# Dyfine/SimCLR_pytorch_distributed

Hardware: AMD Instinct MI355X
Metric: images/sec (whole node) SimCLR ResNet-50 BS=256; CIFAR-10 linear-probe top-1 (higher is better)
Workload: dtype bf16; 1 GPU; model=resnet50 (CIFAR stem) + MLP head 2048-2048-128, SimCLR tau=0.5, global_batch=256, per_gpu_batch=256, views=2, image_size=32, parallelism=dp1, backend=native, syncbn_transport=none, hip_graph=False, loss_steps=254

## Files before the change

csrc/bindings/block_ops.cpp:

```cpp
#include "ops_decl.h"
#include "conv_internal.h"
#include "launchers.h"

namespace sdx_bind {
namespace {

using sdx_plan::knobs;

enum BlockSlot { kOut = 0, kX = 0, kY1, kA1, kY2, kA2, kY3, kYs, kMask, kSlots };
enum BnSlot { kSc = 0, kSh, kMu, kIv, kBnStride };

double rows_of(const torch::Tensor& y) { return (double)(y.numel() / y.size(3)); }

bool sub_addend_enabled() {
  static const bool on = sdx_plan::env_flag("SDX_SUB_ADDEND", true);
  return on;
}

bool dgrad_bnstat_enabled() {
  static const bool on = sdx_plan::env_flag("SDX_DGRAD_BNSTAT", true);
  return on;
}

DgradOpts into(OptT out, OptT addend, OptT addend_mask = {}, int64_t addend_sub = 0) {
  DgradOpts o;
  o.out = out; o.addend = addend; o.addend_mask = addend_mask; o.addend_sub = addend_sub;
  return o;
}

void side_wgrad(const torch::Tensor& dy, const torch::Tensor& x, int64_t R, int64_t S, int64_t stride, int64_t pad,
                const torch::Tensor& sink, int64_t side) {
  if (side == 0) {
    conv_wgrad(dy, x, R, S, stride, pad, 0, -1, sink, true, c10::nullopt, c10::nullopt);
    return;
  }
  auto guard = side_fork(side, dy.device(), {dy, x});
  if (splitk_merge_enabled() && !splitk_deferring(cur_stream())) splitk_defer_begin(cur_stream());
  conv_wgrad(dy, x, R, S, stride, pad, 0, -1, sink, true, c10::nullopt, c10::nullopt);
}

std::vector<torch::Tensor> fold_gram_now(const torch::Tensor& a2) {
  const int64_t K3 = a2.size(3);
  auto opt = a2.options().dtype(at::kFloat);
  auto Sm = torch::empty({K3, 1, 1, K3}, opt);
  conv_wgrad(a2, a2, 1, 1, 1, 0, 0, -1, Sm, false, c10::nullopt, c10::nullopt);
  auto part = torch::empty({bnfold_colsum_blocks(), K3}, opt);
  auto cs = torch::empty({K3}, opt);
  check_hip(launch_bnfold_colsum(a2.data_ptr(), a2.numel() / K3, (int)K3, part.data_ptr<float>(), cs.data_ptr<float>(),
                                 cur_stream()),
            "bnfold_colsum");
  return {Sm, cs, part};
}

std::vector<torch::Tensor> fold_gram(torch::Tensor a2, int64_t side) {
  check_bf16_nhwc(a2, "a2");
  if (side == 0) return fold_gram_now(a2);
  auto guard = side_fork(side, a2.device(), {a2});
  return fold_gram_now(a2);
}

void side_fold_wgrad(const torch::Tensor& dz, const torch::Tensor& a2, const torch::Tensor& w3,
                     const torch::Tensor& coef, const torch::Tensor& sink, int64_t side,
                     const torch::Tensor* gram = nullptr, const torch::Tensor* Gpre = nullptr) {
  if (side != 0 && splitk_deferring(reinterpret_cast<hipStream_t>(side))) check_hip(splitk_flush(), "splitk_flush");
  const int64_t C3 = dz.size(3), K3 = a2.size(3);
  auto body = [&]() {
    auto opt = coef.options();
    torch::Tensor G;
    if (Gpre != nullptr) {
      G = *Gpre;
    } else {
      G = torch::empty({C3, 1, 1, K3}, opt);
      conv_wgrad(dz, a2, 1, 1, 1, 0, 0, -1, G, false, c10::nullopt, c10::nullopt);
    }
    torch::Tensor Sm, cs, part;
    if (gram != nullptr) {
      Sm = gram[0];
      cs = gram[1];
    } else {
      auto g3 = fold_gram_now(a2);
      Sm = g3[0];
      cs = g3[1];
      part = g3[2];
    }
    check_hip(launch_bnfold_wgrad(coef.data_ptr<float>(), G.data_ptr<float>(), Sm.data_ptr<float>(),
                                  cs.data_ptr<float>(), 1, w3.data_ptr(), (int)C3, (int)K3, sink.data_ptr<float>(),
                                  1, cur_stream()),
              "bnfold_wgrad");
    if (side != 0) {
      side_stash().push_back(G);
      side_stash().push_back(Sm);
      side_stash().push_back(cs);
      if (part.defined()) side_stash().push_back(part);
    }
  };
  if (side == 0) {
    body();
    return;
  }
  auto guard = side_fork(side, dz.device(), {dz, a2, w3, coef});
  body();
}

struct FoldOps {
  torch::Tensor w;
  torch::Tensor t;
  torch::Tensor bias;
  bool cat = false;
  DgradOpts dgrad_opts(const torch::Tensor& a2) const {
    DgradOpts o;
    if (cat) {
      o.cat = &a2;
      o.cat_bias = &bias;
    } else {
      o.addend = t;
      o.add_pre = true;
    }
    return o;
  }
};
bool fold_cat_enabled() {
  static const bool on = sdx_plan::env_flag("SDX_FOLD_CAT", true);
  return on;
}
FoldOps fold_dgrad_operands(const torch::Tensor& coef, const torch::Tensor& w3, const torch::Tensor& wt3,
                            const torch::Tensor& a2, const torch::Tensor& mu, const torch::Tensor* gram) {
  const int64_t C3 = w3.size(0), K3 = w3.size(3);
  TORCH_CHECK(w3.size(1) == 1 && w3.size(2) == 1 && wt3.size(0) == K3 && wt3.size(3) == C3 && a2.size(3) == K3 &&
                  coef.numel() == 3 * C3,
              "bn3 fold: conv3 must be 1x1 [C][1][1][K] with a2 of K channels");
  const int64_t rows = a2.numel() / K3;
  TORCH_CHECK(rows < (1LL << 31), "bn3 fold: too many rows");
  check_vec(mu, C3, "fold mu");
  const ConvGeom gd = conv_geom(a2.size(0), a2.size(1), a2.size(2), K3, C3, 1, 1, 1, 0);
  FoldOps r;
  r.bias = torch::empty({K3}, coef.options());
  const float* cs = gram != nullptr ? gram[1].data_ptr<float>() : nullptr;
  if (fold_cat_enabled() && sdx_plan::dgrad_cat_supported(gd, (int)K3, knobs())) {
    r.cat = true;
    r.w = torch::empty({K3, 1, 1, C3 + K3}, w3.options());
    uint16_t* wc = reinterpret_cast<uint16_t*>(r.w.data_ptr());
    check_hip(launch_bnfold_prep(coef.data_ptr<float>(), w3.data_ptr(), wt3.data_ptr(), (int)C3, (int)K3, wc, wc + C3,
                                 r.bias.data_ptr<float>(), mu.data_ptr<float>(), cs, (long)rows, cur_stream(),
                                 (int)(C3 + K3), (int)(C3 + K3)),
              "bnfold_prep");
    return r;
  }
  r.w = torch::empty_like(wt3);
  auto mx = torch::empty({K3, 1, 1, K3}, w3.options());
  check_hip(launch_bnfold_prep(coef.data_ptr<float>(), w3.data_ptr(), wt3.data_ptr(), (int)C3, (int)K3, r.w.data_ptr(),
                               mx.data_ptr(), r.bias.data_ptr<float>(), mu.data_ptr<float>(), cs, (long)rows,
                               cur_stream()),
            "bnfold_prep");
  const ConvGeom g = conv_geom(rows, 1, 1, K3, K3, 1, 1, 1, 0);
  r.t = torch::empty_like(a2);
  const GemmEpi epi{r.bias.data_ptr<float>(), 0, 0};
  check_hip(launch_conv_fwd(g, a2.data_ptr(), mx.data_ptr(), r.t.data_ptr(), nullptr, auto_cfg(rows, K3, K3, true),
                            cur_stream(), nullptr, nullptr, &epi),
            "bnfold T gemm");
  return r;
}

std::vector<torch::Tensor> block_fwd(torch::Tensor x, std::vector<torch::Tensor> w, std::vector<torch::Tensor> bn,
                                     int64_t stride, bool bottleneck, bool proj, bool training, double eps,
                                     double momentum, int64_t comm, bool fold_fwd = false, int64_t side = 0) {
  const int nconv = bottleneck ? 3 : 2;
  TORCH_CHECK((int)w.size() == nconv + (proj ? 1 : 0), "block_fwd: weight count");
  TORCH_CHECK(bn.size() == w.size() * 4, "block_fwd: 4 BN tensors per conv");
  auto bn_fwd = [&](int i, const torch::Tensor& slab, double count) {
    return bn_forward(slab, count, bn[i * 4], bn[i * 4 + 1], bn[i * 4 + 2], bn[i * 4 + 3], eps, momentum, training,
                      comm);
  };
  auto conv_bn = [&](const torch::Tensor& in, int i, int64_t s, int64_t p) -> std::pair<torch::Tensor, BnState> {
    auto c = conv_fwd(in, w[i], s, p, training, -1, c10::nullopt, c10::nullopt);
    return {c[0], bn_fwd(i, c[1], rows_of(c[0]))};
  };
  auto relu_bn = [](const torch::Tensor& y, const BnState& s) {
    return bn_apply(y, s.sc, s.sh, {}, true, c10::nullopt);
  };
  std::vector<BnState> st;
  std::vector<torch::Tensor> out(kMask);
  torch::Tensor ys_side, slab_side;
  hipEvent_t sc_done = nullptr;
  if (proj && training && side != 0) {
    const torch::Tensor& ws = w[nconv];
    check_bf16_nhwc(x, "x");
    check_bf16_nhwc(ws, "w_shortcut");
    TORCH_CHECK(ws.size(3) == x.size(3) && ws.size(1) == 1 && ws.size(2) == 1, "block_fwd: 1x1 shortcut");
    const ConvGeom gs = fwd_geom(x, ws, stride, 0);
    const int64_t M = (int64_t)gs.N * gs.P * gs.Q;
    const int cfg = auto_cfg(M, gs.K, gs.C, true);
    ys_side = torch::empty({gs.N, gs.P, gs.Q, gs.K}, x.options());
    slab_side = torch::empty({sdx_plan::cdiv(M, sdx_plan::tile_m(cfg)), 2, gs.K}, x.options().dtype(at::kFloat));
    auto guard = side_fork(side, x.device(), {});
    check_hip(launch_conv_fwd(gs, x.data_ptr(), ws.data_ptr(), ys_side.data_ptr(), slab_side.data_ptr<float>(), cfg,
                              cur_stream()),
              "block_fwd shortcut conv (side stream)");
    sc_done = stream_mark();
  }
  const int64_t s1 = bottleneck ? 1 : stride, p1 = bottleneck ? 0 : 1;
  auto c1 = conv_bn(x, 0, s1, p1);
  st.push_back(c1.second);
  auto a1 = relu_bn(c1.first, st[0]);
  const int64_t s2 = bottleneck ? stride : 1;
  auto c2 = conv_bn(a1, 1, s2, 1);
  st.push_back(c2.second);
  torch::Tensor last = c2.first, a2;
  int lastbn = 1;
  fold_fwd = fold_fwd && bottleneck && training && w[2].size(1) == 1 && w[2].size(2) == 1 &&
             (proj || (stride == 1 && w[2].size(0) == x.size(3))) && sdx_plan::fwd_bnapply_supported(knobs());
  torch::Tensor o, ys;
  auto shortcut = [&] {
    if (sc_done != nullptr) {
      stream_wait(sc_done);
      st.push_back(bn_fwd(nconv, slab_side, rows_of(ys_side)));
      ys = ys_side;
    } else {
      auto cs = conv_bn(x, nconv, stride, 0);
      st.push_back(cs.second);
      ys = cs.first;
    }
  };
  torch::Tensor omask;
  if (bottleneck) {
    a2 = relu_bn(c2.first, st[1]);
    if (fold_fwd) {
      auto c3s = conv_fwd(a2, w[2], 1, 0, true, -1, c10::nullopt, c10::nullopt, nullptr, true);
      st.push_back(bn_fwd(2, c3s[1], rows_of(a2)));
      GemmEpi epi{};
      epi.bn_scale = st[2].sc.data_ptr<float>();
      epi.bn_shift = st[2].sh.data_ptr<float>();
      if (proj) {
        shortcut();
        TORCH_CHECK(ys.size(0) == a2.size(0) && ys.size(1) == a2.size(1) && ys.size(2) == a2.size(2) &&
                        ys.size(3) == w[2].size(0),
                    "block_fwd: shortcut output shape");
        epi.resid = ys.data_ptr();
        epi.resid_scale = st[3].sc.data_ptr<float>();
        epi.resid_shift = st[3].sh.data_ptr<float>();
      } else {
        epi.resid = x.data_ptr();
      }
      omask = torch::empty({rows_of(a2) * w[2].size(0) / 8}, x.options().dtype(at::kByte));
      epi.mask_out = omask.data_ptr<uint8_t>();
      o = conv_fwd(a2, w[2], 1, 0, false, -1, c10::nullopt, c10::nullopt, &epi)[0];
      last = torch::Tensor();
    } else {
      auto c3 = conv_bn(a2, 2, 1, 0);
      st.push_back(c3.second);
      last = c3.first;
    }
    lastbn = 2;
  }
  if (training && !omask.defined())
    omask = torch::empty({last.numel() / 8}, last.options().dtype(at::kByte));
  const OptT om = training ? OptT(omask) : OptT();
  if (fold_fwd) {
  } else if (proj) {
    shortcut();
    o = bn_apply(last, st[lastbn].sc, st[lastbn].sh, {ys, st[nconv].sc, st[nconv].sh, 1}, true, om);
  } else {
    o = bn_apply(last, st[lastbn].sc, st[lastbn].sh, {x, {}, {}, 2}, true, om);
  }
  out.push_back(omask);
  out[kOut] = o;
  out[kY1] = c1.first;
  out[kA1] = a1;
  out[kY2] = c2.first;
  out[kA2] = bottleneck ? a2 : torch::Tensor();
  out[kY3] = bottleneck ? last : torch::Tensor();
  out[kYs] = ys;
  for (auto& b : st) {
    out.push_back(b.sc);
    out.push_back(b.sh);
    out.push_back(b.mu);
    out.push_back(b.iv);
  }
  return out;
}

std::vector<torch::Tensor> block_bwd(torch::Tensor dout, std::vector<torch::Tensor> saved,
                                     std::vector<torch::Tensor> bnst, std::vector<torch::Tensor> wt,
                                     std::vector<torch::Tensor> dw, std::vector<torch::Tensor> bng, int64_t stride,
                                     bool bottleneck, bool proj, int64_t side, int64_t comm, OptT in_slab,
                                     std::vector<torch::Tensor> prev, std::vector<torch::Tensor> fold_w) {
  const int nconv = bottleneck ? 3 : 2;
  const int nbn = nconv + (proj ? 1 : 0);
  struct DeferGuard {
    bool ok = false;
    ~DeferGuard() {
      if (!ok) splitk_defer_cancel();
    }
  } defer_guard;
  TORCH_CHECK((int)wt.size() == nbn && (int)dw.size() == nbn && (int)bng.size() == 3 * nbn &&
                  (int)bnst.size() == kBnStride * nbn && saved.size() == kSlots,
              "block_bwd: argument counts");
  const torch::Tensor &x = saved[kX], &y1 = saved[kY1], &a1 = saved[kA1], &y2 = saved[kY2], &a2 = saved[kA2],
                      &y3 = saved[kY3], &ys = saved[kYs], &out = saved[kMask];
  auto S = [&](int i, int k) { return bnst[i * kBnStride + k]; };
  auto bset = [&](int i) { return BnBwdSet{bng[i * 3], S(i, kMu), S(i, kIv), bng[i * 3 + 1], bng[i * 3 + 2]}; };
  const int64_t H = x.size(1), W = x.size(2);
  const int lastbn = nconv - 1;
  const torch::Tensor& ylast = bottleneck ? y3 : y2;
  const bool no_y3 = bottleneck && (!y3.defined() || y3.numel() == 0);
  const double cnt_last = rows_of(y2), cnt1 = rows_of(y1);
  torch::Tensor dylast, dys, dz;
  const bool have_slab = in_slab.has_value() && in_slab->defined() && in_slab->numel() > 0;
  if (have_slab) TORCH_CHECK(in_slab->size(1) == (proj ? 3 : 2), "block_bwd: in_slab set count");
  const size_t nfw = fold_w.size() == 3 || fold_w.size() == 6 ? fold_w.size() / 3 : fold_w.size();
  const bool grams = nfw != fold_w.size();
  const bool fold = bottleneck && have_slab && nfw >= 1 && nfw <= (proj ? 2u : 1u) && fold_w[0].defined() &&
                    (nfw == 1 || (stride == 1 && fold_w[1].defined()));
  const bool fold_sc = fold && proj && nfw == 2;
  TORCH_CHECK(!no_y3 || fold, "block_bwd: a forward-folded block needs its BN3 fold (next block's slab)");
  const torch::Tensor* gram3 = grams ? &fold_w[nfw] : nullptr;
  const torch::Tensor* grams_sc = grams && nfw == 2 ? &fold_w[nfw + 2] : nullptr;
  torch::Tensor coef3, coefs, Gfold;
  if (no_y3) {
    const int64_t C3 = dout.size(3), K3 = a2.size(3), ns = in_slab->size(1);
    TORCH_CHECK(in_slab->size(0) > 2 && in_slab->size(2) == C3 && fold_w[0].size(0) == C3 &&
                    fold_w[0].size(3) == K3,
                "block_bwd: forward-folded BN3 slab / weights");
    Gfold = torch::empty({C3, 1, 1, K3}, dout.options().dtype(at::kFloat));
    conv_wgrad(dout, a2, 1, 1, 1, 0, 0, -1, Gfold, false, c10::nullopt, c10::nullopt);
    float* rows = in_slab->data_ptr<float>() + (in_slab->size(0) - 2) * ns * C3;
    check_hip(launch_bnfold_rowdot(Gfold.data_ptr<float>(), fold_w[0].data_ptr(), (int)C3, (int)K3, (int)ns, rows,
                                   cur_stream()),
              "bnfold_rowdot");
  }
  {
    const BnBwdSrc src{dout, out, ylast, proj ? OptT(ys) : OptT()};
    auto c = bn_bwd_coefs(comm, have_slab ? nullptr : &src, have_slab ? &*in_slab : nullptr, cnt_last, bset(lastbn),
                          proj ? bset(nconv) : BnBwdSet{});
    if (fold) {
      coef3 = c[0];
      dz = dout;
      if (fold_sc)
        coefs = c[1];
      else if (proj)
        dys = bn_bwd_apply({dz, {}, ys}, c[1], c10::nullopt, false)[0];
    } else if (proj) {
      auto r = bn_bwd_apply(src, c[0], c[1], false);
      dylast = r[0];
      dys = r[1];
    } else {
      const bool bitmask = out.scalar_type() == at::kByte;
      auto r = bn_bwd_apply(src, c[0], c10::nullopt, !bitmask);
      dylast = r[0];
      dz = bitmask ? torch::Tensor() : r[2];
    }
  }
  auto dgrad_bn = [&](const torch::Tensor& dyo, const torch::Tensor& w, const torch::Tensor& y, int64_t st,
                      int64_t pad, int i, double cnt, const DgradOpts& o = {}) -> std::pair<torch::Tensor, torch::Tensor> {
    if (dgrad_bnstat_enabled()) {
      DgradStat ds;
      ds.ya = y; ds.ma = S(i, kMu); ds.msc = S(i, kSc); ds.msh = S(i, kSh);
      auto r = conv_dgrad_bnstat(dyo, w, y.size(1), y.size(2), st, pad, -1, o, ds);
      return {r[0], bn_bwd_coefs(comm, nullptr, &r[1], cnt, bset(i))[0]};
    }
    auto da = conv_dgrad(dyo, w, y.size(1), y.size(2), st, pad, -1, o);
    const BnBwdSrc src{da, {}, y, {}, S(i, kSc), S(i, kSh)};
    return {da, bn_bwd_coefs(comm, &src, nullptr, cnt, bset(i))[0]};
  };
  auto bn_relu_bwd = [&](const torch::Tensor& da, const torch::Tensor& y, const torch::Tensor& coef, int i) {
    return bn_bwd_apply({da, {}, y, {}, S(i, kSc), S(i, kSh)}, coef, c10::nullopt, false)[0];
  };
  torch::Tensor dy1;
  if (bottleneck) {
    std::pair<torch::Tensor, torch::Tensor> r2;
    if (fold) {
      auto op = fold_dgrad_operands(coef3, fold_w[0], wt[2], a2, S(lastbn, kMu), gram3);
      side_fold_wgrad(dz, a2, fold_w[0], coef3, dw[2], side, gram3, Gfold.defined() ? &Gfold : nullptr);
      r2 = dgrad_bn(dz, op.w, y2, 1, 0, 1, cnt_last, op.dgrad_opts(a2));
    } else {
      side_wgrad(dylast, a2, 1, 1, 1, 0, dw[2], side);
      r2 = dgrad_bn(dylast, wt[2], y2, 1, 0, 1, cnt_last);
    }
    auto dy2 = bn_relu_bwd(r2.first, y2, r2.second, 1);
    side_wgrad(dy2, a1, 3, 3, stride, 1, dw[1], side);
    auto r1 = dgrad_bn(dy2, wt[1], y1, stride, 1, 0, cnt1);
    dy1 = bn_relu_bwd(r1.first, y1, r1.second, 0);
    side_wgrad(dy1, x, 1, 1, 1, 0, dw[0], side);
  } else {
    side_wgrad(dylast, a1, 3, 3, 1, 1, dw[1], side);
    auto r1 = dgrad_bn(dylast, wt[1], y1, 1, 1, 0, cnt1);
    dy1 = bn_relu_bwd(r1.first, y1, r1.second, 0);
    side_wgrad(dy1, x, 3, 3, stride, 1, dw[0], side);
  }
  const int64_t s1 = bottleneck ? 1 : stride, p1 = bottleneck ? 0 : 1;
  const bool want_prev = dgrad_bnstat_enabled() && prev.size() >= 5 && prev[4].defined() && prev[4].numel() > 0;
  const bool prev_fold = want_prev && prev.size() >= 6 && prev[5].defined() && prev[5].numel() > 0;
  torch::Tensor prev_slab;
  auto last_dgrad = [&](const DgradOpts& o) -> torch::Tensor {
    if (!want_prev) return conv_dgrad(dy1, wt[0], H, W, s1, p1, -1, o);
    const bool two = prev[2].defined() && prev[2].numel() > 0;
    const bool prev_noy = !prev[0].defined() || prev[0].numel() == 0;
    TORCH_CHECK(!prev_noy || prev_fold, "block_bwd: previous block without y3 must fold");
    DgradStat ds;
    ds.ya = prev[0]; ds.ma = prev[1]; ds.mask_bits = prev[4];
    if (two) {
      ds.yb = prev[2];
      ds.mb = prev[3];
    }
    ds.store_masked = prev_fold ? 1 : 0;
    ds.extra_rows = prev_noy ? 2 : 0;
    auto r = conv_dgrad_bnstat(dy1, wt[0], H, W, s1, p1, -1, o, ds);
    prev_slab = r[1];
    return r[0];
  };
  torch::Tensor dx;
  if (fold_sc) {
    auto op = fold_dgrad_operands(coefs, fold_w[1], wt[nconv], x, S(nconv, kMu), grams_sc);
    side_fold_wgrad(dz, x, fold_w[1], coefs, dw[nconv], side, grams_sc);
    dx = conv_dgrad(dz, op.w, H, W, 1, 0, -1, op.dgrad_opts(x));
    dx = last_dgrad(into(dx, dx));
  } else if (proj) {
    side_wgrad(dys, x, 1, 1, stride, 0, dw[nconv], side);
    if (stride > 1 && sub_addend_enabled()) {
      auto dxs = conv_dgrad(dys, wt[nconv], dys.size(1), dys.size(2), 1, 0, -1);
      dx = last_dgrad(into({}, dxs, {}, stride));
    } else {
      dx = conv_dgrad(dys, wt[nconv], H, W, stride, 0, -1);
      dx = last_dgrad(into(dx, dx));
    }
  } else if (dz.defined()) {
    dx = last_dgrad(into({}, dz));
  } else {
    dx = last_dgrad(into({}, dout, out));
  }
  check_hip(splitk_flush(), "splitk_flush");
  defer_guard.ok = true;
  return {dx, prev_slab};
}


void check_f32(const torch::Tensor& t, int64_t numel, const char* name) {
  TORCH_CHECK(t.is_cuda() && t.scalar_type() == at::kFloat && t.is_contiguous() && t.numel() == numel, name,
              " must be a contiguous float32 GPU tensor of ", numel, " elements");
}

void check_bf16_flat(const torch::Tensor& t, const char* name) {
  TORCH_CHECK(t.is_cuda() && t.scalar_type() == at::kBFloat16 && t.is_contiguous(), name,
              " must be a contiguous bf16 GPU tensor");
}

std::pair<int64_t, int64_t> fold_weight_dims(const torch::Tensor& w) {
  check_bf16_flat(w, "w");
  TORCH_CHECK(w.dim() == 4 && w.size(1) == 1 && w.size(2) == 1 && w.size(0) > 0 && w.size(3) > 0 &&
                  w.size(0) < (1 << 20) && w.size(3) < (1 << 20),
              "w must be [C][1][1][K]");
  return {w.size(0), w.size(3)};
}

void bnfold_prep_test(torch::Tensor coef, torch::Tensor w, torch::Tensor wt, OptT mu, OptT cs, int64_t rows,
                      int64_t ldw, int64_t ldm, torch::Tensor wd_out, torch::Tensor mx_out, torch::Tensor bias_out) {
  const auto [C, K] = fold_weight_dims(w);
  check_bf16_flat(wt, "wt");
  TORCH_CHECK(wt.dim() == 4 && wt.size(0) == K && wt.size(1) == 1 && wt.size(2) == 1 && wt.size(3) == C,
              "wt must be [K][1][1][C]");
  check_f32(coef, 3 * C, "coef");
  check_f32(bias_out, K, "bias_out");
  check_bf16_flat(wd_out, "wd_out");
  check_bf16_flat(mx_out, "mx_out");
  TORCH_CHECK(rows >= 0 && rows < (1LL << 31) && ldw >= 0 && ldm >= 0 && ldw < (1 << 24) && ldm < (1 << 24),
              "bnfold_prep: rows, ldw or ldm out of range");
  const int64_t lw = ldw == 0 ? C : ldw, lm = ldm == 0 ? K : ldm;
  TORCH_CHECK(wd_out.numel() >= (K - 1) * lw + C, "wd_out too small for K rows of ldw");
  TORCH_CHECK(mx_out.numel() >= (K - 1) * lm + K, "mx_out too small for K rows of ldm");
  const float* pmu = opt_ptr(mu, C, "mu");
  const float* pcs = opt_ptr(cs, K, "cs");
  c10::DeviceGuard dg(w.device());
  check_hip(launch_bnfold_prep(coef.data_ptr<float>(), w.data_ptr(), wt.data_ptr(), (int)C, (int)K, wd_out.data_ptr(),
                               mx_out.data_ptr(), bias_out.data_ptr<float>(), pmu, pcs, (long)rows, cur_stream(),
                               (int)ldw, (int)ldm),
            "bnfold_prep");
}

std::vector<torch::Tensor> bnfold_colsum_test(torch::Tensor x, OptT partial) {
  check_bf16_flat(x, "x");
  TORCH_CHECK(x.dim() == 2 && x.size(1) > 0 && x.numel() < (1LL << 31), "x must be [rows][K] bf16");
  TORCH_CHECK(reinterpret_cast<uintptr_t>(x.data_ptr()) % 16 == 0, "x must be 16-byte aligned");
  const int64_t rows = x.size(0), K = x.size(1);
  c10::DeviceGuard dg(x.device());
  auto opt = x.options().dtype(at::kFloat);
  const int64_t nb = bnfold_colsum_blocks();
  torch::Tensor part = partial.has_value() && partial->defined() ? *partial : torch::empty({nb, K}, opt);
  check_f32(part, nb * K, "partial");
  auto cs = torch::empty({K}, opt);
  check_hip(launch_bnfold_colsum(x.data_ptr(), (long)rows, (int)K, part.data_ptr<float>(), cs.data_ptr<float>(),
                                 cur_stream()),
            "bnfold_colsum");
  return {cs, part};
}

torch::Tensor bnfold_wgrad_test(torch::Tensor coef, torch::Tensor G, torch::Tensor S, torch::Tensor cs,
                                torch::Tensor w, torch::Tensor sink, bool accumulate) {
  const auto [C, K] = fold_weight_dims(w);
  check_f32(coef, 3 * C, "coef");
  check_f32(G, C * K, "G");
  check_f32(S, K * K, "S");
  check_f32(sink, C * K, "sink");
  TORCH_CHECK(cs.dim() == 2 && cs.size(1) == K, "cs must be [ncs][K]");
  check_f32(cs, cs.size(0) * K, "cs");
  c10::DeviceGuard dg(w.device());
  check_hip(launch_bnfold_wgrad(coef.data_ptr<float>(), G.data_ptr<float>(), S.data_ptr<float>(), cs.data_ptr<float>(),
                                (int)cs.size(0), w.data_ptr(), (int)C, (int)K, sink.data_ptr<float>(),
                                accumulate ? 1 : 0, cur_stream()),
            "bnfold_wgrad");
  return sink;
}

torch::Tensor bnfold_rowdot_test(torch::Tensor G, torch::Tensor w, int64_t ns, torch::Tensor out) {
  const auto [C, K] = fold_weight_dims(w);
  check_f32(G, C * K, "G");
  TORCH_CHECK(ns >= 0 && ns <= 16 && out.dim() == 3 && out.size(0) == 2 && out.size(1) == ns && out.size(2) == C,
              "out must be [2][ns][C]");
  check_f32(out, 2 * ns * C, "out");
  c10::DeviceGuard dg(w.device());
  check_hip(launch_bnfold_rowdot(G.data_ptr<float>(), w.data_ptr(), (int)C, (int)K, (int)ns, out.data_ptr<float>(),
                                 cur_stream()),
            "bnfold_rowdot");
  return out;
}

}

void register_block(pybind11::module& m) {
  m.def("bnfold_prep", &bnfold_prep_test, "BN3 fold (test only): Wd, Mx and b into caller-supplied outputs",
        pybind11::arg("coef"), pybind11::arg("w"), pybind11::arg("wt"), pybind11::arg("mu") = pybind11::none(),
        pybind11::arg("cs") = pybind11::none(), pybind11::arg("rows") = 0, pybind11::arg("ldw") = 0,
        pybind11::arg("ldm") = 0, pybind11::arg("wd_out"), pybind11::arg("mx_out"), pybind11::arg("bias_out"));
  m.def("bnfold_colsum", &bnfold_colsum_test, "BN3 fold (test only): column sums of x [rows][K] -> (cs, partial)",
        pybind11::arg("x"), pybind11::arg("partial") = pybind11::none());
  m.def("bnfold_wgrad", &bnfold_wgrad_test, "BN3 fold (test only): the folded weight gradient into sink",
        pybind11::arg("coef"), pybind11::arg("G"), pybind11::arg("S"), pybind11::arg("cs"), pybind11::arg("w"),
        pybind11::arg("sink"), pybind11::arg("accumulate"));
  m.def("bnfold_rowdot", &bnfold_rowdot_test, "BN3 fold (test only): Σ_k W·G as fp32 hi / lo slab rows",
        pybind11::arg("G"), pybind11::arg("w"), pybind11::arg("ns"), pybind11::arg("out"));
  m.def("side_stash_release", [] { side_stash().clear(); },
        "drop the tensors kept alive for side-stream wgrads (after join)");
  m.def("block_fwd", &block_fwd, "native residual-block forward (whole kernel sequence; comm: SyncBN handle or 0)",
        pybind11::arg("x"), pybind11::arg("w"), pybind11::arg("bn"), pybind11::arg("stride"),
        pybind11::arg("bottleneck"), pybind11::arg("proj"), pybind11::arg("training"), pybind11::arg("eps"),
        pybind11::arg("momentum"), pybind11::arg("comm") = 0, pybind11::arg("fold_fwd") = false,
        pybind11::arg("side") = 0);
  m.def("fold_gram", &fold_gram,
        "BN3 fold: [a2ᵀ·a2, Σ_rows a2, scratch] of a folded conv's input, issued on the side stream",
        pybind11::arg("a2"), pybind11::arg("side"));
  m.def("block_bwd", &block_bwd, "native residual-block backward (dgrad chain + side-stream wgrads)",
        pybind11::arg("dout"), pybind11::arg("saved"), pybind11::arg("bnst"), pybind11::arg("wt"),
        pybind11::arg("dw"), pybind11::arg("bng"), pybind11::arg("stride"), pybind11::arg("bottleneck"),
        pybind11::arg("proj"), pybind11::arg("side"), pybind11::arg("comm") = 0,
        pybind11::arg("in_slab") = pybind11::none(), pybind11::arg("prev") = std::vector<torch::Tensor>(),
        pybind11::arg("fold_w") = std::vector<torch::Tensor>());
}

}
```

csrc/bindings/bn_ops.cpp:

```cpp
#include "ops_decl.h"
#include "conv_internal.h"
#include "launchers.h"

#include <map>
#include <mutex>
#include <utility>

namespace sdx_bind {

unsigned* reduce_counters(const torch::Device& dev, int nslots) {
  constexpr int kSlots = 256, kPerSlot = 64;
  TORCH_CHECK(nslots >= 1 && nslots <= kXgmiMaxPeers, "counter slots");
  static std::mutex mu;
  static std::map<int, std::pair<torch::Tensor, int>> pool;
  std::lock_guard<std::mutex> lk(mu);
  auto& e = pool[dev.index()];
  if (!e.first.defined())
    e.first = torch::zeros({kSlots * kPerSlot}, torch::TensorOptions().dtype(at::kInt).device(dev));
  int slot = e.second;
  if (slot + nslots > kSlots) slot = 0;
  e.second = (slot + nslots) % kSlots;
  return reinterpret_cast<unsigned*>(e.first.data_ptr<int>()) + slot * kPerSlot;
}

torch::Tensor reduce_scratch(const torch::Tensor& like, int64_t rows, int64_t nsets, int64_t C, int z) {
  return torch::empty({z * col_reduce_gy((int)rows) * nsets * C}, like.options().dtype(at::kDouble));
}

FusedX fused_exchange(int64_t comm) {
  FusedX f;
  if (comm != 0) f.on = small_comm_fused(comm, &f.x);
  return f;
}

namespace {

struct SyncPlan {
  int world = 1;
  FusedX fx;
  bool rccl() const { return world > 1 && !fx.on; }
  const FusedX* fused() const { return fx.on ? &fx : nullptr; }
};
SyncPlan sync_plan(int64_t comm) {
  SyncPlan p;
  p.world = small_comm_world(comm);
  if (p.world > 1) p.fx = fused_exchange(comm);
  return p;
}

void check_slab(const torch::Tensor& slab, int64_t nsets) {
  TORCH_CHECK(slab.is_cuda() && slab.scalar_type() == at::kFloat && slab.dim() == 3 && slab.size(1) == nsets &&
                  slab.is_contiguous(),
              "slab must be [rows, ", nsets, ", C] float32");
  TORCH_CHECK(slab.size(2) <= 4096, "C <= 4096");
}

torch::Tensor bn_stats_reduce(torch::Tensor slab) {
  check_slab(slab, 2);
  c10::DeviceGuard dg(slab.device());
  const int64_t rows = slab.size(0), C = slab.size(2);
  auto out = torch::empty({2, C}, slab.options().dtype(at::kDouble));
  auto scratch = reduce_scratch(slab, rows, 2, C);
  check_hip(launch_col_reduce(slab.data_ptr<float>(), rows, 2, C, scratch.data_ptr<double>(),
                              reduce_counters(slab.device()), out.data_ptr<double>(), 0, nullptr, nullptr,
                              cur_stream()),
            "bn_stats_reduce");
  return out;
}

struct FinalizeOut {
  torch::Tensor scale, shift, mean, invstd;
};

BnFinalizeArgs finalize_args(const torch::Tensor& like, int64_t C, double count, const OptT& gamma, const OptT& beta,
                             double eps, double momentum, bool update, const OptT& running_mean,
                             const OptT& running_var, FinalizeOut& o) {
  BnFinalizeArgs a{};
  a.count = count;
  a.gamma = opt_ptr(gamma, C, "gamma");
  a.beta = opt_ptr(beta, C, "beta");
  a.eps = (float)eps;
  a.momentum = (float)momentum;
  a.update_running = update ? 1 : 0;
  if (update) {
    TORCH_CHECK(running_mean.has_value() && running_var.has_value(), "running stats required for update");
    check_vec(*running_mean, C, "running_mean");
    check_vec(*running_var, C, "running_var");
    a.running_mean = running_mean->data_ptr<float>();
    a.running_var = running_var->data_ptr<float>();
  }
  auto fo = like.options().dtype(at::kFloat);
  o.scale = torch::empty({C}, fo);
  o.shift = torch::empty({C}, fo);
  o.mean = torch::empty({C}, fo);
  o.invstd = torch::empty({C}, fo);
  a.scale = o.scale.data_ptr<float>();
  a.shift = o.shift.data_ptr<float>();
  a.mean = o.mean.data_ptr<float>();
  a.invstd = o.invstd.data_ptr<float>();
  return a;
}

std::vector<torch::Tensor> bn_finalize(torch::Tensor sums, double count, OptT gamma, OptT beta, double eps,
                                       double momentum, bool update, OptT running_mean, OptT running_var) {
  TORCH_CHECK(sums.is_cuda() && sums.scalar_type() == at::kDouble && sums.dim() == 2 && sums.size(0) == 2 &&
                  sums.is_contiguous(),
              "sums must be [2, C] float64");
  const int64_t C = sums.size(1);
  c10::DeviceGuard dg(sums.device());
  FinalizeOut o;
  const BnFinalizeArgs a =
      finalize_args(sums, C, count, gamma, beta, eps, momentum, update, running_mean, running_var, o);
  check_hip(launch_bn_finalize(sums.data_ptr<double>(), C, a, cur_stream()), "bn_finalize");
  return {o.scale, o.shift, o.mean, o.invstd};
}

std::vector<torch::Tensor> bn_stats_finalize(torch::Tensor slab, double count, OptT gamma, OptT beta, double eps,
                                             double momentum, bool update, OptT running_mean, OptT running_var,
                                             const FusedX* fx = nullptr) {
  check_slab(slab, 2);
  c10::DeviceGuard dg(slab.device());
  const int64_t rows = slab.size(0), C = slab.size(2);
  FinalizeOut o;
  const BnFinalizeArgs a =
      finalize_args(slab, C, count, gamma, beta, eps, momentum, update, running_mean, running_var, o);
  auto sums = torch::empty({2, C}, slab.options().dtype(at::kDouble));
  const int z = fx ? fx->z() : 1;
  auto scratch = reduce_scratch(slab, rows, 2, C, z);
  check_hip(launch_col_reduce(slab.data_ptr<float>(), rows, 2, C, scratch.data_ptr<double>(),
                              reduce_counters(slab.device(), z), sums.data_ptr<double>(), 1, &a, nullptr, cur_stream(),
                              fx ? fx->p() : nullptr),
            "bn_stats_finalize");
  return {o.scale, o.shift, o.mean, o.invstd};
}

std::vector<torch::Tensor> bn_eval_affine(OptT gamma, OptT beta, torch::Tensor rm, torch::Tensor rv, double eps) {
  const int64_t C = rm.numel();
  check_vec(rm, C, "running_mean");
  check_vec(rv, C, "running_var");
  c10::DeviceGuard dg(rm.device());
  auto scale = torch::empty({C}, rm.options()), shift = torch::empty({C}, rm.options());
  check_hip(launch_bn_eval_affine(C, opt_ptr(gamma, C, "gamma"), opt_ptr(beta, C, "beta"), rm.data_ptr<float>(),
                                  rv.data_ptr<float>(), (float)eps, scale.data_ptr<float>(), shift.data_ptr<float>(),
                                  cur_stream()),
            "bn_eval_affine");
  return {scale, shift};
}

}

BnState bn_forward(const torch::Tensor& slab, double count, const torch::Tensor& g, const torch::Tensor& b,
                   const torch::Tensor& rm, const torch::Tensor& rv, double eps, double mom, bool training,
                   int64_t comm) {
  if (!training) {
    auto r = bn_eval_affine(g, b, rm, rv, eps);
    return {r[0], r[1], torch::Tensor(), torch::Tensor()};
  }
  const SyncPlan sp = sync_plan(comm);
  std::vector<torch::Tensor> r;
  if (sp.rccl()) {
    auto sums = bn_stats_reduce(slab);
    small_all_reduce_(comm, sums);
    r = bn_finalize(sums, count * sp.world, g, b, eps, mom, true, rm, rv);
  } else {
    r = bn_stats_finalize(slab, count * sp.world, g, b, eps, mom, true, rm, rv, sp.fused());
    if (sp.fx.on) small_comm_fused_issued(comm);
  }
  return {r[0], r[1], r[2], r[3]};
}

torch::Tensor bn_apply(torch::Tensor y, torch::Tensor scale, torch::Tensor shift, const BnResidual& res, bool relu,
                       OptT mask_out) {
  check_bf16_nhwc(y, "y");
  const int64_t C = y.size(3);
  check_vec(scale, C, "scale");
  check_vec(shift, C, "shift");
  const void* rp = nullptr;
  const float *s2 = nullptr, *t2 = nullptr;
  TORCH_CHECK(res.mode >= 0 && res.mode <= 2, "res_mode");
  if (res.mode != 0) {
    TORCH_CHECK(res.r.has_value(), "residual tensor required");
    check_bf16_nhwc(*res.r, "residual");
    TORCH_CHECK(res.r->sizes() == y.sizes(), "residual shape mismatch");
    rp = res.r->data_ptr();
    if (res.mode == 1) {
      s2 = opt_ptr(res.scale2, C, "scale2");
      t2 = opt_ptr(res.shift2, C, "shift2");
      TORCH_CHECK(s2 && t2, "scale2/shift2 required for res_mode 1");
    }
  }
  c10::DeviceGuard dg(y.device());
  auto out = torch::empty_like(y);
  void* mp = nullptr;
  if (mask_out.has_value()) {
    check_mask(*mask_out, y.numel(), "mask_out");
    mp = mask_out->data_ptr();
  }
  check_hip(launch_bn_apply(y.data_ptr(), scale.data_ptr<float>(), shift.data_ptr<float>(), rp, s2, t2, (int)res.mode,
                            relu ? 1 : 0, out.data_ptr(), y.numel(), C, cur_stream(), mp),
            "bn_apply");
  return out;
}

namespace {

void check_bwd_C(int64_t C) {
  TORCH_CHECK(C <= 2048 && (C & (C - 1)) == 0 && C >= 8, "bn backward supports power-of-two C in [8, 2048]");
}

void mask_source(const BnBwdSrc& s, const void** op, const void** om) {
  if (!s.outv.has_value()) return;
  if (s.outv->scalar_type() == at::kByte) {
    check_mask(*s.outv, s.dout.numel(), "out (bitmask)");
    *om = s.outv->data_ptr();
  } else {
    check_bf16_nhwc(*s.outv, "out");
    TORCH_CHECK(s.outv->sizes() == s.dout.sizes(), "out shape");
    *op = s.outv->data_ptr();
  }
}

struct BwdIn {
  const void* op = nullptr;
  const void* om = nullptr;
  const void* ybp = nullptr;
  const float* map = nullptr;
  const float* mbp = nullptr;
  const float* mk_s = nullptr;
  const float* mk_t = nullptr;
  int64_t C = 0;
  int nsum() const { return ybp ? 3 : 2; }
};

BwdIn bwd_inputs(const BnBwdSrc& s, const BnBwdSet& a, const BnBwdSet& b) {
  BwdIn in;
  check_bf16_nhwc(s.dout, "dout");
  check_bf16_nhwc(s.ya, "ya");
  in.C = s.dout.size(3);
  check_bwd_C(in.C);
  TORCH_CHECK(s.ya.sizes() == s.dout.sizes(), "ya shape");
  check_vec(*a.mean, in.C, "mean_a");
  in.map = a.mean->data_ptr<float>();
  mask_source(s, &in.op, &in.om);
  if (s.yb.has_value()) {
    check_bf16_nhwc(*s.yb, "yb");
    TORCH_CHECK(s.yb->sizes() == s.dout.sizes(), "yb shape");
    TORCH_CHECK(b.mean.has_value(), "mean_b required");
    check_vec(*b.mean, in.C, "mean_b");
    in.ybp = s.yb->data_ptr();
    in.mbp = b.mean->data_ptr<float>();
  }
  in_bn_ptrs(s.msc, s.msh, in.C, &in.mk_s, &in.mk_t);
  return in;
}

torch::Tensor bwd_reduce(const BnBwdSrc& s, const BwdIn& in, const BnCoefArgs* ca, const FusedX* fx, const char* what) {
  const int64_t C = in.C;
  const int nsum = in.nsum();
  const int g = bn_bwd_reduce_blocks(s.dout.numel(), C);
  const int z = fx ? fx->z() : 1;
  auto sums = torch::empty({nsum, C}, s.dout.options().dtype(at::kDouble));
  auto partial = torch::empty({g, nsum, C}, s.dout.options().dtype(at::kFloat));
  auto scratch = reduce_scratch(s.dout, g, nsum, C, z);
  check_hip(launch_bn_bwd_reduce(s.dout.data_ptr(), in.op, s.ya.data_ptr(), in.map, in.ybp, in.mbp, s.dout.numel(), C,
                                 partial.data_ptr<float>(), scratch.data_ptr<double>(),
                                 reduce_counters(s.dout.device(), z), sums.data_ptr<double>(), ca ? 2 : 0, ca,
                                 cur_stream(), in.mk_s, in.mk_t, in.om, fx ? fx->p() : nullptr),
            what);
  return sums;
}

struct CoefOut {
  torch::Tensor coef_a, coef_b, dga, dba, dgb, dbb;
  std::vector<torch::Tensor> list() const { return {coef_a, coef_b, dga, dba, dgb, dbb}; }
};

BnCoefArgs coef_args(const torch::Tensor& like, int64_t C, int nsets, double count, const BnBwdSet& sa,
                     const BnBwdSet& sb, CoefOut& o, double grad_scale) {
  TORCH_CHECK(nsets == 1 || nsets == 2, "1 or 2 BN sets");
  TORCH_CHECK(sa.mean.has_value() && sa.invstd.has_value(), "mean_a/inv_a required");
  check_vec(*sa.mean, C, "mean_a");
  check_vec(*sa.invstd, C, "inv_a");
  auto fo = like.options().dtype(at::kFloat);
  const bool sinks = sa.dgamma_sink.has_value();
  TORCH_CHECK(!sinks || (sa.dbeta_sink.has_value() &&
                         (nsets == 1 || (sb.dgamma_sink.has_value() && sb.dbeta_sink.has_value()))),
              "all gradient sinks must be given together");
  BnCoefArgs a{};
  a.count = count;
  a.accumulate = sinks ? 1 : 0;
  a.grad_scale = grad_scale;
  o.coef_a = torch::empty({3, C}, fo);
  o.dga = sinks ? *sa.dgamma_sink : torch::empty({C}, fo);
  o.dba = sinks ? *sa.dbeta_sink : torch::empty({C}, fo);
  if (sinks) {
    check_vec(o.dga, C, "sink_ga");
    check_vec(o.dba, C, "sink_ba");
  }
  a.g_a = opt_ptr(sa.gamma, C, "g_a");
  a.mean_a = sa.mean->data_ptr<float>();
  a.inv_a = sa.invstd->data_ptr<float>();
  a.coef_a = o.coef_a.data_ptr<float>();
  a.dgamma_a = o.dga.data_ptr<float>();
  a.dbeta_a = o.dba.data_ptr<float>();
  if (nsets == 2) {
    o.coef_b = torch::empty({3, C}, fo);
    o.dgb = sinks ? *sb.dgamma_sink : torch::empty({C}, fo);
    o.dbb = sinks ? *sb.dbeta_sink : torch::empty({C}, fo);
    if (sinks) {
      check_vec(o.dgb, C, "sink_gb");
      check_vec(o.dbb, C, "sink_bb");
    }
    a.g_b = opt_ptr(sb.gamma, C, "g_b");
    a.mean_b = opt_ptr(sb.mean, C, "mean_b");
    a.inv_b = opt_ptr(sb.invstd, C, "inv_b");
    TORCH_CHECK(a.mean_b && a.inv_b, "mean_b/inv_b required");
    a.coef_b = o.coef_b.data_ptr<float>();
    a.dgamma_b = o.dgb.data_ptr<float>();
    a.dbeta_b = o.dbb.data_ptr<float>();
  } else {
    o.coef_b = o.dgb = o.dbb = torch::empty({0}, fo);
  }
  return a;
}

std::vector<torch::Tensor> bn_bwd_coef(torch::Tensor sums, double count, const BnBwdSet& sa, const BnBwdSet& sb,
                                       double grad_scale) {
  TORCH_CHECK(sums.is_cuda() && sums.scalar_type() == at::kDouble && sums.dim() == 2 && sums.is_contiguous(),
              "sums must be [nsets+1, C] float64");
  const int64_t C = sums.size(1);
  const int nsets = (int)sums.size(0) - 1;
  c10::DeviceGuard dg(sums.device());
  CoefOut o;
  const BnCoefArgs a = coef_args(sums, C, nsets, count, sa, sb, o, grad_scale);
  check_hip(launch_bn_bwd_coef(sums.data_ptr<double>(), nsets, C, a, cur_stream()), "bn_bwd_coef");
  return o.list();
}

}

std::vector<torch::Tensor> bn_bwd_coefs(int64_t comm, const BnBwdSrc* src, const torch::Tensor* slab, double count,
                                        const BnBwdSet& sa, const BnBwdSet& sb) {
  TORCH_CHECK((src != nullptr) != (slab != nullptr), "bn_bwd_coefs: one statistics source");
  BwdIn in;
  int64_t rows = 0, nsum, C;
  if (src) {
    in = bwd_inputs(*src, sa, sb);
    nsum = in.nsum();
    C = in.C;
  } else {
    TORCH_CHECK(slab->dim() == 3 && (slab->size(1) == 2 || slab->size(1) == 3), "slab: [rows][2|3][C]");
    check_slab(*slab, slab->size(1));
    rows = slab->size(0); nsum = slab->size(1); C = slab->size(2);
  }
  const torch::Tensor& like = src ? src->dout : *slab;
  c10::DeviceGuard dg(like.device());
  torch::Tensor sums, scratch;
  if (slab) sums = torch::empty({nsum, C}, like.options().dtype(at::kDouble));
  const SyncPlan sp = sync_plan(comm);
  if (slab && !sp.fx.on) scratch = reduce_scratch(like, rows, nsum, C);
  auto slab_reduce = [&](const BnCoefArgs* ca) {
    if (!scratch.defined()) scratch = reduce_scratch(like, rows, nsum, C, sp.fx.z());
    check_hip(launch_col_reduce(slab->data_ptr<float>(), rows, (int)nsum, C, scratch.data_ptr<double>(),
                                reduce_counters(like.device(), sp.fx.z()), sums.data_ptr<double>(), ca ? 2 : 0,
                                nullptr, ca, cur_stream(), sp.fx.p()),
              "bn_bwd_coef_slab");
  };
  if (sp.rccl()) {
    if (src) sums = bwd_reduce(*src, in, nullptr, nullptr, "bn_bwd_reduce");
    else slab_reduce(nullptr);
    small_all_reduce_(comm, sums);
    return bn_bwd_coef(sums, count * sp.world, sa, sb, 1.0 / sp.world);
  }
  CoefOut o;
  const BnCoefArgs a = coef_args(like, C, (int)nsum - 1, count * sp.world, sa, sb, o, 1.0 / sp.world);
  if (src) bwd_reduce(*src, in, &a, sp.fused(), "bn_bwd_reduce_coef");
  else slab_reduce(&a);
  if (sp.fx.on) small_comm_fused_issued(comm);
  return o.list();
}

std::vector<torch::Tensor> bn_bwd_apply(const BnBwdSrc& s, torch::Tensor ca, OptT cb, bool want_dz) {
  const torch::Tensor& dout = s.dout;
  check_bf16_nhwc(dout, "dout");
  check_bf16_nhwc(s.ya, "ya");
  const int64_t C = dout.size(3);
  TORCH_CHECK(s.ya.sizes() == dout.sizes(), "ya shape");
  TORCH_CHECK(ca.is_cuda() && ca.scalar_type() == at::kFloat && ca.numel() == 3 * C && ca.is_contiguous(), "coef_a");
  const void* op = nullptr;
  const void* om = nullptr;
  mask_source(s, &op, &om);
  c10::DeviceGuard dg(dout.device());
  auto dya = torch::empty_like(dout);
  torch::Tensor dyb, dz;
  const void* ybp = nullptr;
  const float* cbp = nullptr;
  if (s.yb.has_value()) {
    check_bf16_nhwc(*s.yb, "yb");
    TORCH_CHECK(s.yb->sizes() == dout.sizes(), "yb shape");
    TORCH_CHECK(cb.has_value() && cb->numel() == 3 * C && cb->scalar_type() == at::kFloat, "coef_b");
    ybp = s.yb->data_ptr();
    cbp = cb->data_ptr<float>();
    dyb = torch::empty_like(dout);
  } else {
    dyb = torch::empty({0}, dout.options());
  }
  const float *mk_s, *mk_t;
  in_bn_ptrs(s.msc, s.msh, C, &mk_s, &mk_t);
  dz = want_dz ? torch::empty_like(dout) : torch::empty({0}, dout.options());
  check_hip(launch_bn_bwd_apply(dout.data_ptr(), op, s.ya.data_ptr(), ca.data_ptr<float>(), ybp, cbp, dya.data_ptr(),
                                ybp ? dyb.data_ptr() : nullptr, want_dz ? dz.data_ptr() : nullptr, dout.numel(), C,
                                cur_stream(), mk_s, mk_t, om),
            "bn_bwd_apply");
  return {dya, dyb, dz};
}

namespace {

torch::Tensor syncbn_exchange_sums(int64_t comm, torch::Tensor slab) {
  FusedX fx = fused_exchange(comm);
  TORCH_CHECK(fx.on, "syncbn_exchange_sums: not a fused (xGMI) communicator of > 1 ranks");
  TORCH_CHECK(slab.is_cuda() && slab.scalar_type() == at::kFloat && slab.is_contiguous(), "slab: contiguous fp32");
  const bool emu = fx.x.mode == 2;
  TORCH_CHECK(slab.dim() == 3 || (emu && slab.dim() == 4), "slab: [rows][nsets][C]",
              emu ? " or [W][rows][nsets][C]" : "");
  if (slab.dim() == 4) TORCH_CHECK(slab.size(0) == fx.x.world, "slab: one block per emulated rank");
  const int64_t rows = slab.size(-3), nsets = slab.size(-2), C = slab.size(-1);
  TORCH_CHECK(nsets >= 1 && nsets <= 3 && C >= 1 && C <= 4096 && rows >= 1, "slab shape");
  if (slab.dim() == 4) fx.x.slab_zstride = (long)(rows * nsets * C);
  c10::DeviceGuard dg(slab.device());
  auto sums = torch::empty({nsets, C}, slab.options().dtype(at::kDouble));
  auto scratch = reduce_scratch(slab, rows, nsets, C, fx.z());
  check_hip(launch_col_reduce(slab.data_ptr<float>(), (int)rows, (int)nsets, (int)C, scratch.data_ptr<double>(),
                              reduce_counters(slab.device(), fx.z()), sums.data_ptr<double>(), 0, nullptr, nullptr,
                              cur_stream(), fx.p()),
            "syncbn_exchange_sums");
  small_comm_fused_issued(comm);
  return sums;
}

}

void register_bn(pybind11::module& m) {
  using T = torch::Tensor;
  m.def("syncbn_exchange_sums", &syncbn_exchange_sums,
        "column reduction + cross-rank exchange of a BN statistics slab in one launch (fused xGMI communicators)");
  m.def("bn_stats_reduce", &bn_stats_reduce);
  m.def("bn_finalize", &bn_finalize);
  m.def("bn_stats_finalize",
        [](T slab, double count, OptT gamma, OptT beta, double eps, double momentum, bool update, OptT running_mean,
           OptT running_var) {
          return bn_stats_finalize(slab, count, gamma, beta, eps, momentum, update, running_mean, running_var);
        },
        "conv stat slab -> BN affine in one launch");
  m.def("bn_eval_affine", &bn_eval_affine);
  m.def("bn_apply",
        [](T y, T scale, T shift, OptT r, OptT scale2, OptT shift2, int64_t res_mode, bool relu, OptT mask_out) {
          return bn_apply(y, scale, shift, BnResidual{r, scale2, shift2, res_mode}, relu, mask_out);
        },
        pybind11::arg("y"), pybind11::arg("scale"), pybind11::arg("shift"),
        pybind11::arg("r") = pybind11::none(), pybind11::arg("scale2") = pybind11::none(),
        pybind11::arg("shift2") = pybind11::none(), pybind11::arg("res_mode") = 0, pybind11::arg("relu") = true,
        pybind11::arg("mask_out") = pybind11::none());
  m.def("bn_bwd_reduce",
        [](T dout, OptT outv, T ya, T ma, OptT yb, OptT mb, OptT msc, OptT msh) {
          const BnBwdSrc s{dout, outv, ya, yb, msc, msh};
          BnBwdSet a, b;
          a.mean = ma;
          b.mean = mb;
          const BwdIn in = bwd_inputs(s, a, b);
          c10::DeviceGuard dg(dout.device());
          return bwd_reduce(s, in, nullptr, nullptr, "bn_bwd_reduce");
        },
        pybind11::arg("dout"), pybind11::arg("outv"), pybind11::arg("ya"),
        pybind11::arg("ma"), pybind11::arg("yb") = pybind11::none(), pybind11::arg("mb") = pybind11::none(),
        pybind11::arg("msc") = pybind11::none(), pybind11::arg("msh") = pybind11::none());
  m.def("bn_bwd_coef",
        [](T sums, double count, OptT g_a, T mean_a, T inv_a, OptT g_b, OptT mean_b, OptT inv_b, OptT sink_ga,
           OptT sink_ba, OptT sink_gb, OptT sink_bb, double grad_scale) {
          return bn_bwd_coef(sums, count, {g_a, mean_a, inv_a, sink_ga, sink_ba}, {g_b, mean_b, inv_b, sink_gb, sink_bb},
                             grad_scale);
        },
        pybind11::arg("sums"), pybind11::arg("count"), pybind11::arg("g_a"),
        pybind11::arg("mean_a"), pybind11::arg("inv_a"), pybind11::arg("g_b") = pybind11::none(),
        pybind11::arg("mean_b") = pybind11::none(), pybind11::arg("inv_b") = pybind11::none(),
        pybind11::arg("sink_ga") = pybind11::none(), pybind11::arg("sink_ba") = pybind11::none(),
        pybind11::arg("sink_gb") = pybind11::none(), pybind11::arg("sink_bb") = pybind11::none(),
        pybind11::arg("grad_scale") = 1.0);
  m.def("bn_bwd_reduce_coef",
        [](T dout, OptT outv, T ya, T ma, OptT yb, OptT mb, OptT msc, OptT msh, double count, OptT g_a, T inv_a,
           OptT g_b, OptT inv_b, OptT sink_ga, OptT sink_ba, OptT sink_gb, OptT sink_bb) {
          const BnBwdSrc s{dout, outv, ya, yb, msc, msh};
          return bn_bwd_coefs(0, &s, nullptr, count, {g_a, ma, inv_a, sink_ga, sink_ba},
                              {g_b, mb, inv_b, sink_gb, sink_bb});
        },
        pybind11::arg("dout"), pybind11::arg("outv"),
        pybind11::arg("ya"), pybind11::arg("ma"), pybind11::arg("yb") = pybind11::none(),
        pybind11::arg("mb") = pybind11::none(), pybind11::arg("msc") = pybind11::none(),
        pybind11::arg("msh") = pybind11::none(), pybind11::arg("count") = 1.0, pybind11::arg("g_a") = pybind11::none(),
        pybind11::arg("inv_a") = pybind11::none(), pybind11::arg("g_b") = pybind11::none(),
        pybind11::arg("inv_b") = pybind11::none(), pybind11::arg("sink_ga") = pybind11::none(),
        pybind11::arg("sink_ba") = pybind11::none(), pybind11::arg("sink_gb") = pybind11::none(),
        pybind11::arg("sink_bb") = pybind11::none());
  m.def("bn_bwd_coef_slab",
        [](int64_t comm, T slab, double count, OptT g_a, T mean_a, T inv_a, OptT g_b, OptT mean_b, OptT inv_b,
           OptT sink_ga, OptT sink_ba, OptT sink_gb, OptT sink_bb) {
          return bn_bwd_coefs(comm, nullptr, &slab, count, {g_a, mean_a, inv_a, sink_ga, sink_ba},
                              {g_b, mean_b, inv_b, sink_gb, sink_bb});
        },
        "BN-backward coefficients (+dγ/dβ into sinks) from a dgrad stat slab",
        pybind11::arg("comm"), pybind11::arg("slab"), pybind11::arg("count"), pybind11::arg("g_a"),
        pybind11::arg("mean_a"), pybind11::arg("inv_a"), pybind11::arg("g_b") = pybind11::none(),
        pybind11::arg("mean_b") = pybind11::none(), pybind11::arg("inv_b") = pybind11::none(),
        pybind11::arg("sink_ga") = pybind11::none(), pybind11::arg("sink_ba") = pybind11::none(),
        pybind11::arg("sink_gb") = pybind11::none(), pybind11::arg("sink_bb") = pybind11::none());
  m.def("bn_bwd_apply",
        [](T dout, OptT outv, T ya, T ca, OptT yb, OptT cb, bool want_dz, OptT msc, OptT msh) {
          return bn_bwd_apply(BnBwdSrc{dout, outv, ya, yb, msc, msh}, ca, cb, want_dz);
        },
        pybind11::arg("dout"), pybind11::arg("outv"), pybind11::arg("ya"),
        pybind11::arg("ca"), pybind11::arg("yb") = pybind11::none(), pybind11::arg("cb") = pybind11::none(),
        pybind11::arg("want_dz") = false, pybind11::arg("msc") = pybind11::none(),
        pybind11::arg("msh") = pybind11::none());
}

}
```

csrc/include/bn_epilogue.h:

```cpp
#pragma once
#include "launchers.h"

namespace sdx {
__device__ __forceinline__ void bn_finalize_one(int c, double s1, double s2, const BnFinalizeArgs& a) {
  const double mean = s1 / a.count;
  double var = s2 / a.count - mean * mean;
  if (var < 0.0) var = 0.0;
  const float invstd = (float)(1.0 / sqrt(var + (double)a.eps));
  const float g = a.gamma ? a.gamma[c] : 1.f;
  const float b = a.beta ? a.beta[c] : 0.f;
  a.scale[c] = g * invstd;
  a.shift[c] = b - (float)mean * g * invstd;
  a.mean[c] = (float)mean;
  a.invstd[c] = invstd;
  if (a.update_running) {
    const double unbiased = a.count > 1.0 ? var * a.count / (a.count - 1.0) : var;
    a.running_mean[c] = (1.f - a.momentum) * a.running_mean[c] + a.momentum * (float)mean;
    a.running_var[c] = (1.f - a.momentum) * a.running_var[c] + a.momentum * (float)unbiased;
  }
}

__device__ __forceinline__ void bn_coef_one(int c, int C, const double* s, int nsets, const BnCoefArgs& a) {
  const double sdz = s[0];
  for (int set = 0; set < nsets; ++set) {
    const float* gg = set == 0 ? a.g_a : a.g_b;
    const float* mm = set == 0 ? a.mean_a : a.mean_b;
    const float* iv = set == 0 ? a.inv_a : a.inv_b;
    float* coef = set == 0 ? a.coef_a : a.coef_b;
    const double sdzy = s[1 + set];
    const double inv = iv[c], mu = mm[c], gam = gg ? gg[c] : 1.0;
    const double A = gam * inv;
    const double m1 = sdz / a.count, m2 = sdzy / a.count;
    const double D = -A * inv * inv * m2;
    const double E = -A * m1 - D * mu;
    coef[c] = (float)A;
    coef[C + c] = (float)D;
    coef[2 * C + c] = (float)E;
    float* dg = set == 0 ? a.dgamma_a : a.dgamma_b;
    float* db = set == 0 ? a.dbeta_a : a.dbeta_b;
    if (dg) dg[c] = (float)(sdzy * inv * a.grad_scale) + (a.accumulate ? dg[c] : 0.f);
    if (db) db[c] = (float)(sdz * a.grad_scale) + (a.accumulate ? db[c] : 0.f);
  }
}

}
```

csrc/include/conv_internal.h:

```cpp
#pragma once
#include <torch/extension.h>

#include <c10/hip/HIPGuard.h>

#include <initializer_list>
#include <vector>

#include "launchers.h"

namespace sdx_bind {
using OptT = c10::optional<torch::Tensor>;

void check_bf16_nhwc(const torch::Tensor& t, const char* name);
void check_vec(const torch::Tensor& t, int64_t C, const char* name);
const float* opt_ptr(const OptT& t, int64_t C, const char* name);
void in_bn_ptrs(const OptT& sc, const OptT& sh, int64_t C, const float** ps, const float** pt);
void check_mask(const torch::Tensor& m, int64_t numel, const char* name);

ConvGeom conv_geom(int64_t N, int64_t H, int64_t W, int64_t C, int64_t K, int64_t R, int64_t S, int64_t stride,
                   int64_t pad);
ConvGeom fwd_geom(const torch::Tensor& x, const torch::Tensor& w, int64_t stride, int64_t pad);
ConvGeom dgrad_geom(const torch::Tensor& dy, const torch::Tensor& wt, int64_t H, int64_t W, int64_t stride,
                    int64_t pad);
int auto_cfg(int64_t M, int64_t Ncol, int64_t Kdim = 0, bool fill = false);

std::vector<torch::Tensor> conv_fwd(torch::Tensor x, torch::Tensor w, int64_t stride, int64_t pad, bool want_stats,
                                    int64_t cfg, OptT in_scale, OptT in_shift, const GemmEpi* epi = nullptr,
                                    bool no_out = false);
struct DgradOpts {
  OptT out, addend, addend_mask;
  int64_t addend_sub = 0;
  bool add_pre = false;
  const torch::Tensor* cat = nullptr;
  const torch::Tensor* cat_bias = nullptr;
};
struct DgradStat {
  torch::Tensor ya, ma;
  OptT yb, mb, mask_bits, msc, msh;
  int store_masked = 0;
  int64_t extra_rows = 0;
};
torch::Tensor conv_dgrad(torch::Tensor dy, torch::Tensor wt, int64_t H, int64_t W, int64_t stride, int64_t pad,
                         int64_t cfg, const DgradOpts& o = {});
std::vector<torch::Tensor> conv_dgrad_bnstat(torch::Tensor dy, torch::Tensor wt, int64_t H, int64_t W,
                                             int64_t stride, int64_t pad, int64_t cfg, const DgradOpts& o,
                                             const DgradStat& st);
torch::Tensor conv_wgrad(torch::Tensor dy, torch::Tensor x, int64_t R, int64_t S, int64_t stride, int64_t pad,
                         int64_t splits, int64_t cfg, OptT out, bool accumulate, OptT in_scale, OptT in_shift);
bool splitk_merge_enabled();

unsigned* reduce_counters(const torch::Device& dev, int nslots = 1);
torch::Tensor reduce_scratch(const torch::Tensor& like, int64_t rows, int64_t nsets, int64_t C, int z = 1);
struct FusedX {
  XgmiCol x{};
  bool on = false;
  int z() const { return on && x.mode == 2 && !x.solo ? x.world : 1; }
  const XgmiCol* p() const { return on ? &x : nullptr; }
};
FusedX fused_exchange(int64_t comm);

struct BnState {
  torch::Tensor sc, sh, mu, iv;
};
BnState bn_forward(const torch::Tensor& slab, double count, const torch::Tensor& g, const torch::Tensor& b,
                   const torch::Tensor& rm, const torch::Tensor& rv, double eps, double mom, bool training,
                   int64_t comm);
struct BnResidual {
  OptT r, scale2, shift2;
  int64_t mode = 0;
};
torch::Tensor bn_apply(torch::Tensor y, torch::Tensor scale, torch::Tensor shift, const BnResidual& res, bool relu,
                       OptT mask_out);
struct BnBwdSet {
  OptT gamma, mean, invstd, dgamma_sink, dbeta_sink;
};
struct BnBwdSrc {
  torch::Tensor dout;
  OptT outv;
  torch::Tensor ya;
  OptT yb, msc, msh;
};
std::vector<torch::Tensor> bn_bwd_coefs(int64_t comm, const BnBwdSrc* src, const torch::Tensor* slab, double count,
                                        const BnBwdSet& a, const BnBwdSet& b = {});
std::vector<torch::Tensor> bn_bwd_apply(const BnBwdSrc& s, torch::Tensor ca, OptT cb, bool want_dz);

std::vector<torch::Tensor>& side_stash();
hipEvent_t stream_mark();
void stream_wait(hipEvent_t ev);
c10::hip::HIPStreamGuard side_fork(int64_t side, const torch::Device& dev, std::initializer_list<torch::Tensor> keep);
}
```

csrc/include/launchers.h:

```cpp
#pragma once
#include <hip/hip_runtime.h>
#include <stdint.h>

#include "conv_plan.h"

hipError_t launch_mfma16_selftest(const void* A, const void* B, float* C, hipStream_t s);

hipError_t launch_rownorm_fwd(const float* x, int N, int D, float eps, float* y, float* norms, hipStream_t s);
hipError_t launch_rownorm_bwd(const float* dy, const float* y, const float* norms, int N, int D, float eps, float* dx,
                              hipStream_t s);
hipError_t launch_norm_stats(const float* x, int N, int D, int mode, double* sums, double n_global, float momentum,
                             float* rec, float* valid, float* out, hipStream_t s);

bool linear_ce_supported(int K, int C);
hipError_t launch_linear_ce_fwd(const float* x, const float* W, const float* bias, const int64_t* labels, int B,
                                int K, int C, float gscale, float* logits, float* dz, float* rowstat, hipStream_t s,
                                const int64_t* rows = nullptr, long N = 0);
hipError_t launch_linear_ce_fwd_soft(const float* x, const float* W, const float* bias, const int64_t* labels,
                                     const int64_t* labels2, float lam, float eps, int B, int K, int C, float gscale,
                                     float* logits, float* dz, float* rowstat, hipStream_t s);
hipError_t launch_linear_ce_sgd(const float* x, const float* dz, int B, int K, int C, float* W, float* bias,
                                float* bufW, float* bufb, float lr, float mom, float wd, int first,
                                const float* rowstat, float* stats, hipStream_t s, const int64_t* rows = nullptr,
                                long N = 0);
hipError_t launch_ce_head_bwd(const float* x, const float* dz, const float* W, int B, int K, int C, const float* gout,
                              float* dX, float* dW, float* db, const float* rowstat, float* stats, float* loss,
                              hipStream_t s);

bool head_gemm_supported(int G, int B, int K, int C);
hipError_t launch_head_gemm_logits(const float* x, const float* W, const float* bias, const int64_t* labels, int G,
                                   int B, int K, int C, float gscale, float* logits, float* dz, float* rowstat,
                                   hipStream_t s, const int64_t* rows = nullptr, long N = 0);
hipError_t launch_head_gemm_logits_soft(const float* x, const float* W, const float* bias, const int64_t* labels,
                                        const int64_t* labels2, float lam, float eps, int B, int K, int C,
                                        float gscale, float* logits, float* dz, float* rowstat, hipStream_t s);
hipError_t launch_head_gemm_stats(int G, int B, int K, int C, const float* rowstat, float* stats, float* loss,
                                  hipStream_t s);
hipError_t launch_head_gemm_sgd(const float* x, const float* dz, int G, int B, int K, int C, float* W, float* bias,
                                float* bufW, float* bufb, const float* lrs, const float* wds, float mom, int first,
                                const float* rowstat, float* stats, hipStream_t s, const int64_t* rows = nullptr,
                                long N = 0);
hipError_t launch_head_gemm_bwd(const float* x, const float* dz, const float* W, int B, int K, int C,
                                const float* gout, float* dX, float* dW, float* db, const float* rowstat,
                                float* stats, float* loss, hipStream_t s);

constexpr int kLinearSweepMaxHeads = 16;
bool linear_ce_sweep_supported(int G, int K, int C);
hipError_t launch_linear_ce_sweep_fwd(const float* x, const float* W, const float* bias, const int64_t* labels, int G,
                                      int B, int K, int C, float gscale, float* logits, float* dz, float* rowstat,
                                      hipStream_t s, const int64_t* rows = nullptr, long N = 0);
hipError_t launch_linear_ce_sweep_sgd(const float* x, const float* dz, int G, int B, int K, int C, float* W,
                                      float* bias, float* bufW, float* bufb, const float* lrs, const float* wds,
                                      float mom, int first, const float* rowstat, float* stats, hipStream_t s,
                                      const int64_t* rows = nullptr, long N = 0);

int supcon_num_splits(int n_own, int n_other);
hipError_t launch_supcon_fwd(const float* A, const float* C, const int* a_self, const int* a_key,
                             const int* c_key, int Na, int N, int D, float inv_temp, float temp_ratio,
                             float scale, int n_split, float* part, float* lse, float* invcnt,
                             float* row_loss, float* loss, hipStream_t s);
long supcon_bwd_workspace(int Na, int N, int D);
long supcon_bwd_sum_workspace(int N, int D);
hipError_t launch_supcon_bwd_sum(const float* X, const int* a_self, const int* a_key, const int* c_key,
                                 const float* lse, const float* invcnt, int N, int D, float inv_temp, float w,
                                 const float* gscale, float* dX, float* ws, hipStream_t s);
hipError_t launch_supcon_bwd(const float* A, const float* C, const int* a_self, const int* a_key,
                             const int* c_key, const float* lse, const float* invcnt, int Na, int N, int D,
                             float inv_temp, float w, const float* gscale, float* dA, float* dC, float* ws,
                             hipStream_t s);

hipError_t launch_bnfold_prep(const float* coef, const void* w, const void* wt, int C, int K, void* wd, void* mx,
                              float* bias, const float* mu, const float* cs, long rows, hipStream_t s, int ldw = 0,
                              int ldm = 0);
hipError_t launch_bnfold_wgrad(const float* coef, const float* G, const float* S, const float* cs, int ncs,
                               const void* w, int C, int K, float* sink, int accumulate, hipStream_t s);
int bnfold_colsum_blocks();
hipError_t launch_bnfold_rowdot(const float* G, const void* w, int C, int K, int ns, float* out_rows, hipStream_t s);
hipError_t launch_bnfold_colsum(const void* x, long rows, int K, float* partial, float* cs, hipStream_t s);

struct BnBwdStat {
  float* slab;
  const void* ya;
  const float* ma;
  const void* yb;
  const float* mb;
  const uint8_t* mask;
  const float* msc;
  const float* msh;
  int row0;
  int store_masked;
};
struct GemmEpi {
  const float* bias;
  int relu;
  int out_f32;
  int add_pre;
  const float* bn_scale;
  const float* bn_shift;
  const void* resid;
  uint8_t* mask_out;
  const float* resid_scale;
  const float* resid_shift;
  const void* cat_a;
  int cat_ch;
  const float* bias_pre;
};
int igemm_trace_slots();
hipError_t igemm_trace_copy(unsigned long long* host, hipStream_t s);
hipError_t launch_conv_fwd(const ConvGeom& g, const void* x, const void* w, void* y, float* stats, int cfg,
                           hipStream_t s, const float* in_scale = nullptr, const float* in_shift = nullptr,
                           const GemmEpi* epi = nullptr);
hipError_t launch_conv_dgrad_class(const ConvGeom& g, int ph, int pw, const void* dy, const void* wt, void* dx,
                                   const void* addend, int cfg, hipStream_t s, const void* addend_mask = nullptr,
                                   const BnBwdStat* bstat = nullptr, int addend_sub = 0,
                                   const GemmEpi* epi = nullptr);
hipError_t launch_conv_dgrad_merged(const ConvGeom& g, const sdx_plan::DgradPlan& plan, const void* dy, const void* wt,
                                    void* dx, const void* addend, hipStream_t s, const void* addend_mask = nullptr,
                                    const BnBwdStat* bstat = nullptr, int addend_sub = 0);
hipError_t launch_conv_wgrad(const ConvGeom& g, const sdx_plan::WgradPlan& plan, const void* dy, const void* x,
                             float* partial, float* dw, int accumulate, hipStream_t s,
                             const float* in_scale = nullptr, const float* in_shift = nullptr);
hipError_t launch_splitk_reduce(const float* partial, int splits, long n4, float* dw, int accumulate, hipStream_t s);
void splitk_defer_begin(hipStream_t s);
bool splitk_deferring(hipStream_t s);
hipError_t splitk_flush();
void splitk_defer_cancel();
hipError_t launch_wgrad3x3(const ConvGeom& g, const sdx_plan::WgradPlan& plan, const void* dy, const void* x,
                           float* partial, float* dw, int accumulate, hipStream_t s);
hipError_t launch_wgrad1x1(const ConvGeom& g, const sdx_plan::WgradPlan& plan, const void* dy, const void* x,
                           float* partial, float* dw, int accumulate, hipStream_t s);

struct BnFinalizeArgs {
  double count;
  const float* gamma;
  const float* beta;
  float eps, momentum;
  int update_running;
  float* running_mean;
  float* running_var;
  float *scale, *shift, *mean, *invstd;
};
struct BnCoefArgs {
  double count;
  const float *g_a, *mean_a, *inv_a, *g_b, *mean_b, *inv_b;
  float *coef_a, *coef_b, *dgamma_a, *dbeta_a, *dgamma_b, *dbeta_b;
  int accumulate;
  double grad_scale = 1.0;
};
constexpr int kXgmiMaxPeers = 8;
constexpr int kXgmiFlagGroups = 64;
struct XgmiPeers {
  double* data[kXgmiMaxPeers];
  unsigned* flags[kXgmiMaxPeers];
  size_t cap;
};
struct XgmiCol {
  XgmiPeers peers;
  int mode = 0, me = 0, world = 1;
  unsigned epoch = 0;
  unsigned* epoch_ctr = nullptr;
  int* err = nullptr;
  long long timeout_ticks = 0;
  long slab_zstride = 0;
  int solo = 0;
};

int col_reduce_gy(int rows);
hipError_t launch_col_reduce(const float* slab, int rows, int nsets, int C, double* scratch, unsigned* counters,
                             double* sums, int epi, const BnFinalizeArgs* fa, const BnCoefArgs* ca, hipStream_t s,
                             const XgmiCol* xg = nullptr);
hipError_t launch_bn_finalize(const double* sums, int C, const BnFinalizeArgs& a, hipStream_t s);
hipError_t launch_bn_eval_affine(int C, const float* gamma, const float* beta, const float* rm, const float* rv,
                                 float eps, float* scale, float* shift, hipStream_t s);
hipError_t launch_bn_apply(const void* y, const float* sc, const float* sh, const void* r, const float* sc2,
                           const float* sh2, int res_mode, int relu, void* out, long numel, int C, hipStream_t s,
                           void* mask_out = nullptr);
int bn_bwd_reduce_blocks(long numel, int C);
hipError_t launch_bn_bwd_reduce(const void* dout, const void* outv, const void* ya, const float* ma, const void* yb,
                                const float* mb, long numel, int C, float* partial, double* scratch,
                                unsigned* counters, double* sums, int epi, const BnCoefArgs* ca, hipStream_t s,
                                const float* msc = nullptr, const float* msh = nullptr, const void* omask = nullptr,
                                const XgmiCol* xg = nullptr);
hipError_t launch_bn_bwd_coef(const double* sums, int nsets, int C, const BnCoefArgs& a, hipStream_t s);
hipError_t launch_bn_bwd_apply(const void* dout, const void* outv, const void* ya, const float* ca, const void* yb,
                               const float* cb, void* dya, void* dyb, void* dz_out, long numel, int C, hipStream_t s,
                               const float* msc = nullptr, const float* msh = nullptr, const void* omask = nullptr);

hipError_t launch_gpu_augment(const uint8_t* data, const int64_t* idx, int B, int H, int W, int S, int n_views,
                              uint64_t seed, const float* mean, const float* std, float scale_lo, float scale_hi,
                              float ratio_lo, float ratio_hi, float jitter_p, float bright, float contrast,
                              float sat, float hue, float gray_p, int do_crop, int do_flip, const int64_t* seed_dev,
                              void* out, hipStream_t s, long n_data = 0, const int64_t* offs = nullptr,
                              const int32_t* hw = nullptr);
hipError_t launch_gpu_augment_blur(const uint8_t* data, const int64_t* idx, int B, int H, int W, int S, int n_views,
                                   uint64_t seed, const float* mean, const float* std, float scale_lo,
                                   float scale_hi, float ratio_lo, float ratio_hi, float jitter_p, float bright,
                                   float contrast, float sat, float hue, float gray_p, int do_crop, int do_flip,
                                   float blur_p, int blur_k, float sigma_lo, float sigma_hi, int rows,
                                   const int64_t* seed_dev, void* out, hipStream_t s, long n_data = 0,
                                   const int64_t* offs = nullptr, const int32_t* hw = nullptr);
hipError_t launch_gpu_eval_crop(const uint8_t* data, const int64_t* idx, int B, int H, int W, int S, int R,
                                const float* mean, const float* std, void* out, hipStream_t s, long n_data = 0,
                                const int64_t* offs = nullptr, const int32_t* hw = nullptr);

enum MixMode { kMixMixup = 1, kMixCutmix = 2 };
hipError_t launch_mix_views(const void* x, void* out, int B, int H, int W, int mode, float lam, int y0, int y1, int x0,
                            int x1, hipStream_t s);

hipError_t launch_sgd(float* p, const float* g, float* buf, long n, const float* lr, float momentum, float wd,
                      float gscale, int nesterov, hipStream_t s, int max_blocks = 0);
hipError_t launch_lars(float* p, const float* g, float* buf, const long* seg_off, const int* adapt, int nseg, long n,
                       const float* lr, float momentum, float wd, float gscale, float eta, float* norms,
                       float* part, hipStream_t s);

hipError_t launch_maxpool_fwd(const void* x, void* y, int N, int H, int W, int C, int P, int Q, int k, int stride,
                              int pad, hipStream_t s);
hipError_t launch_maxpool_bwd(const void* x, const void* y, const void* dy, void* dx, int N, int H, int W, int C,
                              int P, int Q, int k, int stride, int pad, hipStream_t s);
hipError_t launch_maxpool_fwd_idx(const void* x, void* y, uint8_t* idx, int N, int H, int W, int C, int P, int Q,
                                  int k, int stride, int pad, hipStream_t s);
hipError_t launch_maxpool_bwd_idx(const uint8_t* idx, const void* dy, void* dx, int N, int H, int W, int C, int P,
                                  int Q, int k, int stride, int pad, hipStream_t s);
hipError_t launch_gap_fwd(const void* x, float* y, int N, int HW, int C, hipStream_t s);
hipError_t launch_gap_bwd(const float* dy, void* dx, int N, int HW, int C, hipStream_t s);

hipError_t launch_wprep(const float* master, void* out, const void* segs, int nseg, long total, hipStream_t s);
hipError_t launch_unpad_add(const float* src, float* dst, int rows, int Cp, int C, hipStream_t s);

hipError_t launch_xgmi_allreduce(const double* in, double* out, int n, const XgmiPeers& peers, int me, int world,
                                 unsigned epoch, int* err, long long timeout_ticks, hipStream_t s,
                                 unsigned* epoch_ctr = nullptr);
hipError_t launch_gpu_stall(long long ticks, hipStream_t s);
hipError_t launch_xgmi_emulate(const double* in, double* out, int n, const XgmiPeers& peers, int world,
                               unsigned epoch, int* err, hipStream_t s);
```

csrc/kernels/bn.hip:

```cpp
#include <cstdlib>

#include "common.h"
#include "launchers.h"
#include "bn_epilogue.h"

using namespace sdx;

namespace {

#ifndef SDX_EW_UNROLL
#define SDX_EW_UNROLL 1
#endif
#ifndef SDX_CR_UNROLL
#define SDX_CR_UNROLL 8
#endif

template <int NS, int XG>
__device__ bool xg_exchange(double (&t)[NS], int c, int C, const XgmiCol& xg, int me) {
  constexpr int kScope = XG == 1 ? __HIP_MEMORY_SCOPE_SYSTEM : __HIP_MEMORY_SCOPE_AGENT;
  const int W = xg.world;
  unsigned* ctr = xg.epoch_ctr != nullptr ? xg.epoch_ctr + 2 * (XG == 2 ? me : 0) : nullptr;
  __shared__ unsigned ep_s;
  if (threadIdx.x == 0)
    ep_s = ctr != nullptr ? __hip_atomic_load(ctr, __ATOMIC_RELAXED, __HIP_MEMORY_SCOPE_AGENT) + 1u : xg.epoch;
  __syncthreads();
  const unsigned epoch = ep_s;
  const int par = epoch & 1;
  const size_t cap = xg.peers.cap;
  __shared__ int ok;
  if (threadIdx.x < 64 && c < C) {
    for (int p = 0; p < W; ++p) {
      unsigned long long* dst =
          reinterpret_cast<unsigned long long*>(xg.peers.data[p] + ((size_t)par * W + me) * cap);
#pragma unroll
      for (int q = 0; q < NS; ++q)
        __hip_atomic_store(dst + (size_t)q * C + c, (unsigned long long)__double_as_longlong(t[q]), __ATOMIC_RELAXED,
                           kScope);
    }
  }
  asm volatile("s_waitcnt vmcnt(0)" ::: "memory");
  if (threadIdx.x == 0) ok = 1;
  __syncthreads();
  if (threadIdx.x < W) {
    const int p = threadIdx.x;
    __hip_atomic_store(xg.peers.flags[p] + ((size_t)par * W + me) * kXgmiFlagGroups + blockIdx.x, epoch,
                       __ATOMIC_RELAXED, kScope);
  }
  if (threadIdx.x < W && !(XG == 2 && xg.solo && threadIdx.x != me)) {
    const int p = threadIdx.x;
    unsigned* f = xg.peers.flags[me] + ((size_t)par * W + p) * kXgmiFlagGroups + blockIdx.x;
    const long long t0 = wall_clock64();
    unsigned spins = 0;
    while (__hip_atomic_load(f, __ATOMIC_RELAXED, kScope) != epoch) {
      if ((++spins & 63) == 0 && wall_clock64() - t0 > xg.timeout_ticks) {
        atomicExch(&ok, 0);
        if (xg.err) __hip_atomic_store(xg.err, 1 + p, __ATOMIC_RELAXED, __HIP_MEMORY_SCOPE_SYSTEM);
        break;
      }
      __builtin_amdgcn_s_sleep(1);
    }
  }
  __syncthreads();
  if (ctr != nullptr && threadIdx.x == 0) {
    const unsigned t = __hip_atomic_fetch_add(ctr + 1, 1u, __ATOMIC_RELAXED, __HIP_MEMORY_SCOPE_AGENT);
    if (t == gridDim.x - 1) {
      __hip_atomic_store(ctr + 1, 0u, __ATOMIC_RELAXED, __HIP_MEMORY_SCOPE_AGENT);
      __hip_atomic_store(ctr, epoch, __ATOMIC_RELAXED, __HIP_MEMORY_SCOPE_AGENT);
    }
  }
  if (!ok) return false;
  if (threadIdx.x < 64 && c < C) {
    const unsigned long long* base =
        reinterpret_cast<const unsigned long long*>(xg.peers.data[me] + (size_t)par * W * cap);
#pragma unroll
    for (int q = 0; q < NS; ++q) {
      double v = 0.0;
      for (int p = 0; p < W; ++p)
        v += __longlong_as_double(
            (long long)__hip_atomic_load(base + (size_t)p * cap + (size_t)q * C + c, __ATOMIC_RELAXED, kScope));
      t[q] = v;
    }
  }
  return true;
}

template <int NS, int EPI, int XG>
__global__ __launch_bounds__(256) void col_reduce_kernel(const float* __restrict__ slab, int rows, int C,
                                                         double* scratch, unsigned* counters,
                                                         double* __restrict__ sums, BnFinalizeArgs fa, BnCoefArgs ca,
                                                         XgmiCol xg) {
  __shared__ double red[NS][4][64];
  __shared__ int is_last;
  const int tx = threadIdx.x & 63, ty = threadIdx.x >> 6;
  const int vz = XG == 2 ? (int)blockIdx.z : 0;
  if constexpr (XG == 2) {
    slab += (size_t)vz * xg.slab_zstride;
    scratch += (size_t)vz * gridDim.y * NS * C;
    counters += vz * 64;
  }
  const int c = blockIdx.x * 64 + tx;
  const int gy = gridDim.y;
  const int per = (rows + gy - 1) / gy;
  const int r0 = blockIdx.y * per, r1 = min(rows, r0 + per);
  double acc[NS];
#pragma unroll
  for (int q = 0; q < NS; ++q) acc[q] = 0.0;
  if (c < C) {
    constexpr int U = SDX_CR_UNROLL;
    int r = r0 + ty;
    for (; r + 4 * (U - 1) < r1; r += 4 * U) {
      float v[U][NS];
#pragma unroll
      for (int u = 0; u < U; ++u)
#pragma unroll
        for (int q = 0; q < NS; ++q) v[u][q] = slab[((size_t)(r + 4 * u) * NS + q) * C + c];
#pragma unroll
      for (int u = 0; u < U; ++u)
#pragma unroll
        for (int q = 0; q < NS; ++q) acc[q] += (double)v[u][q];
    }
    for (; r < r1; r += 4)
#pragma unroll
      for (int q = 0; q < NS; ++q) acc[q] += (double)slab[((size_t)r * NS + q) * C + c];
  }
#pragma unroll
  for (int q = 0; q < NS; ++q) red[q][ty][tx] = acc[q];
  __syncthreads();
  unsigned long long* sc = reinterpret_cast<unsigned long long*>(scratch);
  if (ty == 0 && c < C) {
#pragma unroll
    for (int q = 0; q < NS; ++q) {
      const double v = red[q][0][tx] + red[q][1][tx] + red[q][2][tx] + red[q][3][tx];
      __hip_atomic_store(sc + ((size_t)blockIdx.y * NS + q) * C + c, (unsigned long long)__double_as_longlong(v),
                         __ATOMIC_RELAXED, __HIP_MEMORY_SCOPE_AGENT);
    }
  }
  if (gy > 1) {
    asm volatile("s_waitcnt vmcnt(0)" ::: "memory");
    __syncthreads();
    if (threadIdx.x == 0) {
      const unsigned t = __hip_atomic_fetch_add(counters + blockIdx.x, 1u, __ATOMIC_RELAXED, __HIP_MEMORY_SCOPE_AGENT);
      is_last = (t == (unsigned)gy - 1u);
    }
    __syncthreads();
    if (!is_last) return;
  }
  {
    double t[NS];
#pragma unroll
    for (int q = 0; q < NS; ++q) t[q] = 0.0;
    if (c < C) {
      constexpr int MAXY = 16;
      unsigned long long v[MAXY][NS];
#pragma unroll
      for (int k = 0; k < MAXY; ++k) {
        const int y = ty + 4 * k;
        if (y < gy) {
#pragma unroll
          for (int q = 0; q < NS; ++q)
            v[k][q] = __hip_atomic_load(sc + ((size_t)y * NS + q) * C + c, __ATOMIC_RELAXED,
                                        __HIP_MEMORY_SCOPE_AGENT);
        }
      }
#pragma unroll
      for (int k = 0; k < MAXY; ++k)
        if (ty + 4 * k < gy)
#pragma unroll
          for (int q = 0; q < NS; ++q) t[q] += __longlong_as_double((long long)v[k][q]);
    }
    __syncthreads();
#pragma unroll
    for (int q = 0; q < NS; ++q) red[q][ty][tx] = t[q];
    __syncthreads();
  }
  double t[NS];
#pragma unroll
  for (int q = 0; q < NS; ++q) t[q] = red[q][0][tx] + red[q][1][tx] + red[q][2][tx] + red[q][3][tx];
  bool go = true;
  if constexpr (XG != 0) go = xg_exchange<NS, XG>(t, c, C, xg, XG == 2 ? vz : xg.me);
  if (go && ty == 0 && c < C && vz == 0) {
#pragma unroll
    for (int q = 0; q < NS; ++q) sums[(size_t)q * C + c] = t[q];
    if constexpr (EPI == 1) bn_finalize_one(c, t[0], t[1], fa);
    if constexpr (EPI == 2) bn_coef_one(c, C, t, NS - 1, ca);
    if constexpr (EPI == 3) ca.dbeta_a[c] += (float)(t[0] * ca.grad_scale);
  }
  if (gy > 1 && threadIdx.x == 0) __hip_atomic_store(counters + blockIdx.x, 0u, __ATOMIC_RELAXED, __HIP_MEMORY_SCOPE_AGENT);
}

__global__ void bn_finalize_kernel(const double* __restrict__ sums, int C, BnFinalizeArgs a) {
  const int c = blockIdx.x * blockDim.x + threadIdx.x;
  if (c < C) bn_finalize_one(c, sums[c], sums[C + c], a);
}

__global__ void bn_eval_affine_kernel(int C, const float* __restrict__ gamma, const float* __restrict__ beta,
                                      const float* __restrict__ rm, const float* __restrict__ rv, float eps,
                                      float* __restrict__ scale, float* __restrict__ shift) {
  const int c = blockIdx.x * blockDim.x + threadIdx.x;
  if (c >= C) return;
  const float invstd = rsqrtf(rv[c] + eps);
  const float g = gamma ? gamma[c] : 1.f;
  scale[c] = g * invstd;
  shift[c] = (beta ? beta[c] : 0.f) - rm[c] * g * invstd;
}

__device__ __forceinline__ void load8c(const float* __restrict__ p, float (&v)[8]) {
  const float4 a = reinterpret_cast<const float4*>(p)[0], b = reinterpret_cast<const float4*>(p)[1];
  v[0] = a.x; v[1] = a.y; v[2] = a.z; v[3] = a.w; v[4] = b.x; v[5] = b.y; v[6] = b.z; v[7] = b.w;
}

__device__ __forceinline__ uint8_t relu_bits(uint4 v) {
  const uint32_t w[4] = {v.x, v.y, v.z, v.w};
  uint32_t b = 0;
#pragma unroll
  for (int q = 0; q < 4; ++q) {
    const uint32_t lo = w[q] & 0xffffu, hi = w[q] >> 16;
    b |= (uint32_t)((lo & 0x7fffu) != 0 && !(lo & 0x8000u)) << (2 * q);
    b |= (uint32_t)((hi & 0x7fffu) != 0 && !(hi & 0x8000u)) << (2 * q + 1);
  }
  return (uint8_t)b;
}

template <int RES, bool RELU>
struct ApplyOp {
  float ss[8], tt[8], aa[8], bb[8];
  __device__ __forceinline__ void load(const float* sc, const float* sh, const float* sc2, const float* sh2, int c0) {
    load8c(sc + c0, ss);
    load8c(sh + c0, tt);
    if (RES == 1) {
      load8c(sc2 + c0, aa);
      load8c(sh2 + c0, bb);
    }
  }
  __device__ __forceinline__ uint4 run(uint4 yv, uint4 rv4) const {
    float v[8];
    unpack8(yv, v);
#pragma unroll
    for (int i = 0; i < 8; ++i) v[i] = v[i] * ss[i] + tt[i];
    if (RES != 0) {
      float rv[8];
      unpack8(rv4, rv);
#pragma unroll
      for (int i = 0; i < 8; ++i) v[i] += RES == 1 ? rv[i] * aa[i] + bb[i] : rv[i];
    }
    if (RELU) {
#pragma unroll
      for (int i = 0; i < 8; ++i) v[i] = fmaxf(v[i], 0.f);
    }
    return pack8(v);
  }
};

template <int RES, bool RELU>
__global__ __launch_bounds__(256) void bn_apply_kernel(const uint16_t* __restrict__ y, const float* __restrict__ sc,
                                                       const float* __restrict__ sh, const uint16_t* __restrict__ r,
                                                       const float* __restrict__ sc2, const float* __restrict__ sh2,
                                                       uint16_t* __restrict__ out, long n8l, int C8,
                                                       uint8_t* __restrict__ mask_out) {
  const int n8 = (int)n8l, stride = gridDim.x * blockDim.x;
  const int e0 = blockIdx.x * blockDim.x + threadIdx.x;
  const uint4* Y = reinterpret_cast<const uint4*>(y);
  const uint4* R = reinterpret_cast<const uint4*>(r);
  uint4* O = reinterpret_cast<uint4*>(out);
  ApplyOp<RES, RELU> op;
  if ((stride % C8) == 0) {
    op.load(sc, sh, sc2, sh2, (e0 % C8) * 8);
    int e = e0;
    for (; e + (SDX_EW_UNROLL - 1) * stride < n8; e += SDX_EW_UNROLL * stride) {
      uint4 yv[SDX_EW_UNROLL], rv[SDX_EW_UNROLL];
#pragma unroll
      for (int u = 0; u < SDX_EW_UNROLL; ++u) {
        yv[u] = ld16s<SDX_NT_EW_LOAD != 0>(Y + e + u * stride);
        rv[u] = RES != 0 ? ld16s<SDX_NT_EW_LOAD != 0>(R + e + u * stride) : make_uint4(0, 0, 0, 0);
      }
#pragma unroll
      for (int u = 0; u < SDX_EW_UNROLL; ++u) {
        const uint4 o = op.run(yv[u], rv[u]);
        st16<SDX_NT_EW != 0>(O + e + u * stride, o);
        if (mask_out) mask_out[e + u * stride] = relu_bits(o);
      }
    }
    for (; e < n8; e += stride) {
      const uint4 o = op.run(ld16s<SDX_NT_EW_LOAD != 0>(Y + e),
                             RES != 0 ? ld16s<SDX_NT_EW_LOAD != 0>(R + e) : make_uint4(0, 0, 0, 0));
      st16<SDX_NT_EW != 0>(O + e, o);
      if (mask_out) mask_out[e] = relu_bits(o);
    }
  } else {
    for (int e = e0; e < n8; e += stride) {
      op.load(sc, sh, sc2, sh2, (e % C8) * 8);
      const uint4 o = op.run(Y[e], RES != 0 ? R[e] : make_uint4(0, 0, 0, 0));
      O[e] = o;
      if (mask_out) mask_out[e] = relu_bits(o);
    }
  }
}

template <bool TWO>
__global__ __launch_bounds__(256) void bn_bwd_reduce_kernel(const uint16_t* __restrict__ dout,
                                                            const uint16_t* __restrict__ outv,
                                                            const uint16_t* __restrict__ ya, const float* __restrict__ ma,
                                                            const uint16_t* __restrict__ yb, const float* __restrict__ mb,
                                                            long n8, int C8, int C, float* __restrict__ partial,
                                                            const float* __restrict__ msc,
                                                            const float* __restrict__ msh,
                                                            const uint8_t* __restrict__ omask) {
  constexpr int NS = TWO ? 3 : 2;
  __shared__ float red[NS][256][8];
  const long tid = blockIdx.x * (long)blockDim.x + threadIdx.x;
  const long stride = (long)gridDim.x * blockDim.x;
  const int grp = (int)(tid % C8);
  const int c0 = grp * 8;
  float mua[8], mub[8];
#pragma unroll
  for (int i = 0; i < 8; ++i) {
    mua[i] = ma[c0 + i];
    mub[i] = TWO ? mb[c0 + i] : 0.f;
  }
  const bool mask_y = outv == nullptr && omask == nullptr && msc != nullptr;
  float mks[8], mkt[8];
#pragma unroll
  for (int i = 0; i < 8; ++i) {
    mks[i] = mask_y ? msc[c0 + i] : 0.f;
    mkt[i] = mask_y ? msh[c0 + i] : 0.f;
  }
  float s0[8] = {0}, s1[8] = {0}, s2[8] = {0};
  const uint4* D = reinterpret_cast<const uint4*>(dout);
  const uint4* OV = reinterpret_cast<const uint4*>(outv);
  const uint4* YA = reinterpret_cast<const uint4*>(ya);
  const uint4* YB = reinterpret_cast<const uint4*>(yb);
  auto accum = [&](uint4 dv, uint4 ov, uint4 av, uint4 bv, uint32_t mbits) {
    float d[8], a[8];
    unpack8(dv, d);
    unpack8(av, a);
    if (omask) {
#pragma unroll
      for (int i = 0; i < 8; ++i) d[i] = (mbits >> i) & 1u ? d[i] : 0.f;
    } else if (outv) {
      float o[8];
      unpack8(ov, o);
#pragma unroll
      for (int i = 0; i < 8; ++i) d[i] = o[i] > 0.f ? d[i] : 0.f;
    } else if (mask_y) {
#pragma unroll
      for (int i = 0; i < 8; ++i) d[i] = a[i] * mks[i] + mkt[i] > 0.f ? d[i] : 0.f;
    }
#pragma unroll
    for (int i = 0; i < 8; ++i) {
      s0[i] += d[i];
      s1[i] += d[i] * (a[i] - mua[i]);
    }
    if (TWO) {
      float b[8];
      unpack8(bv, b);
#pragma unroll
      for (int i = 0; i < 8; ++i) s2[i] += d[i] * (b[i] - mub[i]);
    }
  };
  const uint4 z = make_uint4(0, 0, 0, 0);
  for (long e = tid; e < n8; e += stride)
    accum(D[e], outv ? OV[e] : z, YA[e], TWO ? YB[e] : z, omask ? (uint32_t)omask[e] : 0u);
#pragma unroll
  for (int i = 0; i < 8; ++i) {
    red[0][threadIdx.x][i] = s0[i];
    red[1][threadIdx.x][i] = s1[i];
    if (TWO) red[NS - 1][threadIdx.x][i] = s2[i];
  }
  __syncthreads();
  if ((int)threadIdx.x < C8 && C8 <= 256) {
    double acc[NS][8];
#pragma unroll
    for (int q = 0; q < NS; ++q)
#pragma unroll
      for (int i = 0; i < 8; ++i) acc[q][i] = 0.0;
    for (int t = threadIdx.x; t < 256; t += C8)
#pragma unroll
      for (int q = 0; q < NS; ++q)
#pragma unroll
        for (int i = 0; i < 8; ++i) acc[q][i] += red[q][t][i];
    const int g0 = (int)threadIdx.x * 8;
#pragma unroll
    for (int q = 0; q < NS; ++q)
#pragma unroll
      for (int i = 0; i < 8; ++i) partial[((size_t)blockIdx.x * NS + q) * C + g0 + i] = (float)acc[q][i];
  }
}

__global__ void bn_bwd_coef_kernel(const double* __restrict__ sums, int nsets, int C, BnCoefArgs a) {
  const int c = blockIdx.x * blockDim.x + threadIdx.x;
  if (c >= C) return;
  double t[3];
  for (int q = 0; q <= nsets; ++q) t[q] = sums[(size_t)q * C + c];
  bn_coef_one(c, C, t, nsets, a);
}

template <bool TWO>
struct BwdApplyOp {
  float A[8], Dc[8], E[8], B2[8], D2[8], E2[8], ms[8], mt[8];
  bool use_mask;
  __device__ __forceinline__ void load(const float* ca, const float* cb, const float* msc, const float* msh, int C,
                                       int c0) {
    load8c(ca + c0, A);
    load8c(ca + C + c0, Dc);
    load8c(ca + 2 * C + c0, E);
    if (TWO) {
      load8c(cb + c0, B2);
      load8c(cb + C + c0, D2);
      load8c(cb + 2 * C + c0, E2);
    }
    use_mask = msc != nullptr;
    if (use_mask) {
      load8c(msc + c0, ms);
      load8c(msh + c0, mt);
    }
  }
  __device__ __forceinline__ void run(uint4 dv, uint4 ov, bool has_out, uint4 av, uint4 bv, float (&d)[8],
                                      uint4& ra, uint4& rb, const uint8_t* omask, int e) const {
    float a[8], r[8];
    unpack8(dv, d);
    unpack8(av, a);
    if (omask) {
      const uint32_t mb = omask[e];
#pragma unroll
      for (int i = 0; i < 8; ++i) d[i] = (mb >> i) & 1u ? d[i] : 0.f;
    } else if (has_out) {
      float o[8];
      unpack8(ov, o);
#pragma unroll
      for (int i = 0; i < 8; ++i) d[i] = o[i] > 0.f ? d[i] : 0.f;
    } else if (use_mask) {
#pragma unroll
      for (int i = 0; i < 8; ++i) d[i] = a[i] * ms[i] + mt[i] > 0.f ? d[i] : 0.f;
    }
#pragma unroll
    for (int i = 0; i < 8; ++i) r[i] = A[i] * d[i] + Dc[i] * a[i] + E[i];
    ra = pack8(r);
    if (TWO) {
      unpack8(bv, a);
#pragma unroll
      for (int i = 0; i < 8; ++i) r[i] = B2[i] * d[i] + D2[i] * a[i] + E2[i];
      rb = pack8(r);
    }
  }
};

template <bool TWO>
__global__ __launch_bounds__(256) void bn_bwd_apply_kernel(const uint16_t* __restrict__ dout,
                                                           const uint16_t* __restrict__ outv,
                                                           const uint16_t* __restrict__ ya, const float* __restrict__ ca,
                                                           const uint16_t* __restrict__ yb, const float* __restrict__ cb,
                                                           uint16_t* __restrict__ dya, uint16_t* __restrict__ dyb,
                                                           uint16_t* __restrict__ dz_out, long n8l, int C8, int C,
                                                           const float* __restrict__ msc,
                                                           const float* __restrict__ msh,
                                                           const uint8_t* __restrict__ omask) {
  const int n8 = (int)n8l, stride = gridDim.x * blockDim.x;
  const int e0 = blockIdx.x * blockDim.x + threadIdx.x;
  const uint4* D = reinterpret_cast<const uint4*>(dout);
  const uint4* OV = reinterpret_cast<const uint4*>(outv);
  const uint4* YA = reinterpret_cast<const uint4*>(ya);
  const uint4* YB = reinterpret_cast<const uint4*>(yb);
  uint4* DA = reinterpret_cast<uint4*>(dya);
  uint4* DB = reinterpret_cast<uint4*>(dyb);
  uint4* DZ = reinterpret_cast<uint4*>(dz_out);
  const bool has_out = outv != nullptr;
  const uint4 z = make_uint4(0, 0, 0, 0);
  BwdApplyOp<TWO> op;
  auto one = [&](int e, uint4 dv, uint4 ov, uint4 av, uint4 bv) {
    float d[8];
    uint4 ra, rb;
    op.run(dv, ov, has_out, av, bv, d, ra, rb, omask, e);
    if (DZ) st16<SDX_NT_EW != 0>(DZ + e, pack8(d));
    st16<SDX_NT_EW != 0>(DA + e, ra);
    if (TWO) st16<SDX_NT_EW != 0>(DB + e, rb);
  };
  if ((stride % C8) == 0) {
    op.load(ca, cb, msc, msh, C, (e0 % C8) * 8);
    int e = e0;
    for (; e + (SDX_EW_UNROLL - 1) * stride < n8; e += SDX_EW_UNROLL * stride) {
      uint4 dv[SDX_EW_UNROLL], ov[SDX_EW_UNROLL], av[SDX_EW_UNROLL], bv[SDX_EW_UNROLL];
#pragma unroll
      for (int u = 0; u < SDX_EW_UNROLL; ++u) {
        const int eu = e + u * stride;
        dv[u] = ld16s<SDX_NT_EW_LOAD != 0>(D + eu);
        ov[u] = has_out ? ld16s<SDX_NT_EW_LOAD != 0>(OV + eu) : z;
        av[u] = ld16s<SDX_NT_EW_LOAD != 0>(YA + eu);
        bv[u] = TWO ? ld16s<SDX_NT_EW_LOAD != 0>(YB + eu) : z;
      }
#pragma unroll
      for (int u = 0; u < SDX_EW_UNROLL; ++u) one(e + u * stride, dv[u], ov[u], av[u], bv[u]);
    }
    for (; e < n8; e += stride)
      one(e, ld16s<SDX_NT_EW_LOAD != 0>(D + e), has_out ? ld16s<SDX_NT_EW_LOAD != 0>(OV + e) : z,
          ld16s<SDX_NT_EW_LOAD != 0>(YA + e), TWO ? ld16s<SDX_NT_EW_LOAD != 0>(YB + e) : z);
  } else {
    for (int e = e0; e < n8; e += stride) {
      op.load(ca, cb, msc, msh, C, (e % C8) * 8);
      one(e, D[e], has_out ? OV[e] : z, YA[e], TWO ? YB[e] : z);
    }
  }
}

int ew_grid(long n8, bool bwd = false) {
  auto env_cap = [](const char* name, long dflt) {
    const long v = (long)sdx_plan::env_int(name, 0);
    return v >= 8 ? v / 8 * 8 : dflt;
  };
  static const long cap_fwd = env_cap("SDX_EW_BLOCKS", 2048L);
  static const long cap_bwd = env_cap("SDX_EW_BLOCKS_BWD", cap_fwd);
  const long cap = bwd ? cap_bwd : cap_fwd;
  long g = (n8 + 256L * SDX_EW_UNROLL - 1) / (256L * SDX_EW_UNROLL);
  if (g > cap) g = cap;
  if (g < 1) g = 1;
  return (int)g;
}

}

int col_reduce_gy(int rows) {
  static const double scale = [] {
    const char* e = sdx_plan::env_str("SDX_CR_GY");
    const double v = e ? atof(e) : 0.0;
    return v > 0.0 ? v : 0.5;
  }();
  int gy = (int)(sqrt((double)rows) * scale + 0.5);
  if (gy > 64) gy = 64;
  if (gy < 1) gy = 1;
  return gy;
}

hipError_t launch_col_reduce(const float* slab, int rows, int nsets, int C, double* scratch, unsigned* counters,
                             double* sums, int epi, const BnFinalizeArgs* fa, const BnCoefArgs* ca, hipStream_t s,
                             const XgmiCol* xg) {
  if (rows < 1 || C < 1 || (epi == 1 && (nsets != 2 || !fa)) || (epi == 2 && (nsets < 2 || !ca)) ||
      (epi == 3 && (nsets > 2 || !ca || !ca->dbeta_a)) || (nsets == 1 && epi != 0 && epi != 3))
    return hipErrorInvalidValue;
  const int xm = xg ? xg->mode : 0;
  if (xg && (xm < 1 || xm > 2 || xg->world < 1 || xg->world > kXgmiMaxPeers || xg->me < 0 || xg->me >= xg->world ||
             (size_t)nsets * C > xg->peers.cap || (C + 63) / 64 > kXgmiFlagGroups || xg->timeout_ticks <= 0))
    return hipErrorInvalidValue;
  if (xg && xm == 2 && xg->slab_zstride < 0) return hipErrorInvalidValue;
  if (xg && xm == 2 && !xg->solo && ((C + 63) / 64) * xg->world > 512) return hipErrorInvalidValue;
  if (xg && xg->solo && (xm != 2 || xg->me != 0)) return hipErrorInvalidValue;
  const dim3 grid((C + 63) / 64, col_reduce_gy(rows), xm == 2 && !xg->solo ? xg->world : 1), blk(256);
  const BnFinalizeArgs f = fa ? *fa : BnFinalizeArgs{};
  const BnCoefArgs k = ca ? *ca : BnCoefArgs{};
  const XgmiCol x = xg ? *xg : XgmiCol{};
#define SDX_CR(NS, EPI)                                                                                              \
  do {                                                                                                               \
    if (xm == 0)                                                                                                     \
      hipLaunchKernelGGL((col_reduce_kernel<NS, EPI, 0>), grid, blk, 0, s, slab, rows, C, scratch, counters, sums, f, \
                         k, x);                                                                                      \
    else if (xm == 1)                                                                                                \
      hipLaunchKernelGGL((col_reduce_kernel<NS, EPI, 1>), grid, blk, 0, s, slab, rows, C, scratch, counters, sums, f, \
                         k, x);                                                                                      \
    else                                                                                                             \
      hipLaunchKernelGGL((col_reduce_kernel<NS, EPI, 2>), grid, blk, 0, s, slab, rows, C, scratch, counters, sums, f, \
                         k, x);                                                                                      \
  } while (0)
  if (nsets == 1) {
    if (epi == 0) SDX_CR(1, 0); else SDX_CR(1, 3);
  } else if (nsets == 2) {
    if (epi == 0) SDX_CR(2, 0); else if (epi == 1) SDX_CR(2, 1); else if (epi == 2) SDX_CR(2, 2); else SDX_CR(2, 3);
  } else if (nsets == 3) {
    if (epi == 0) SDX_CR(3, 0); else SDX_CR(3, 2);
  } else {
    return hipErrorInvalidValue;
  }
#undef SDX_CR
  SDX_LAUNCH_CHECK();
  return hipSuccess;
}

hipError_t launch_bn_finalize(const double* sums, int C, const BnFinalizeArgs& a, hipStream_t s) {
  hipLaunchKernelGGL(bn_finalize_kernel, dim3((C + 255) / 256), dim3(256), 0, s, sums, C, a);
  SDX_LAUNCH_CHECK();
  return hipSuccess;
}

hipError_t launch_bn_eval_affine(int C, const float* gamma, const float* beta, const float* rm, const float* rv,
                                 float eps, float* scale, float* shift, hipStream_t s) {
  hipLaunchKernelGGL(bn_eval_affine_kernel, dim3((C + 255) / 256), dim3(256), 0, s, C, gamma, beta, rm, rv, eps,
                     scale, shift);
  SDX_LAUNCH_CHECK();
  return hipSuccess;
}

hipError_t launch_bn_apply(const void* y, const float* sc, const float* sh, const void* r, const float* sc2,
                           const float* sh2, int res_mode, int relu, void* out, long numel, int C, hipStream_t s,
                           void* mask_out) {
  const long n8 = numel / 8;
  const int C8 = C / 8;
  const dim3 grid(ew_grid(n8)), blk(256);
  const uint16_t* yy = (const uint16_t*)y;
  const uint16_t* rr = (const uint16_t*)r;
  uint16_t* oo = (uint16_t*)out;
#define SDX_APPLY(RM, RL) \
  hipLaunchKernelGGL((bn_apply_kernel<RM, RL>), grid, blk, 0, s, yy, sc, sh, rr, sc2, sh2, oo, n8, C8, (uint8_t*)mask_out)
  if (res_mode == 0) { if (relu) SDX_APPLY(0, true); else SDX_APPLY(0, false); }
  else if (res_mode == 1) { if (relu) SDX_APPLY(1, true); else SDX_APPLY(1, false); }
  else { if (relu) SDX_APPLY(2, true); else SDX_APPLY(2, false); }
#undef SDX_APPLY
  SDX_LAUNCH_CHECK();
  return hipSuccess;
}

int bn_bwd_reduce_blocks(long numel, int C) {
  const long n8 = numel / 8;
  long g = (n8 + 256 * 16 - 1) / (256 * 16);
  if (g > 1024) g = 1024;
  if (g < 1) g = 1;
  (void)C;
  return (int)g;
}

hipError_t launch_bn_bwd_reduce(const void* dout, const void* outv, const void* ya, const float* ma, const void* yb,
                                const float* mb, long numel, int C, float* partial, double* scratch,
                                unsigned* counters, double* sums, int epi, const BnCoefArgs* ca, hipStream_t s,
                                const float* msc, const float* msh, const void* omask, const XgmiCol* xg) {
  const int nsets = yb ? 3 : 2;
  const long n8 = numel / 8;
  const int C8 = C / 8;
  const int g = bn_bwd_reduce_blocks(numel, C);
  if (yb)
    hipLaunchKernelGGL((bn_bwd_reduce_kernel<true>), dim3(g), dim3(256), 0, s, (const uint16_t*)dout,
                       (const uint16_t*)outv, (const uint16_t*)ya, ma, (const uint16_t*)yb, mb, n8, C8, C, partial,
                       msc, msh, (const uint8_t*)omask);
  else
    hipLaunchKernelGGL((bn_bwd_reduce_kernel<false>), dim3(g), dim3(256), 0, s, (const uint16_t*)dout,
                       (const uint16_t*)outv, (const uint16_t*)ya, ma, (const uint16_t*)nullptr, (const float*)nullptr,
                       n8, C8, C, partial, msc, msh, (const uint8_t*)omask);
  SDX_LAUNCH_CHECK();
  if (xg && xg->mode == 2 && xg->slab_zstride != 0) return hipErrorInvalidValue;
  return launch_col_reduce(partial, g, nsets, C, scratch, counters, sums, epi, nullptr, ca, s, xg);
}

hipError_t launch_bn_bwd_coef(const double* sums, int nsets, int C, const BnCoefArgs& a, hipStream_t s) {
  hipLaunchKernelGGL(bn_bwd_coef_kernel, dim3((C + 255) / 256), dim3(256), 0, s, sums, nsets, C, a);
  SDX_LAUNCH_CHECK();
  return hipSuccess;
}

hipError_t launch_bn_bwd_apply(const void* dout, const void* outv, const void* ya, const float* ca, const void* yb,
                               const float* cb, void* dya, void* dyb, void* dz_out, long numel, int C, hipStream_t s,
                               const float* msc, const float* msh, const void* omask) {
  const long n8 = numel / 8;
  const int C8 = C / 8;
  if (yb)
    hipLaunchKernelGGL((bn_bwd_apply_kernel<true>), dim3(ew_grid(n8, true)), dim3(256), 0, s, (const uint16_t*)dout,
                       (const uint16_t*)outv, (const uint16_t*)ya, ca, (const uint16_t*)yb, cb, (uint16_t*)dya,
                       (uint16_t*)dyb, (uint16_t*)dz_out, n8, C8, C, msc, msh, (const uint8_t*)omask);
  else
    hipLaunchKernelGGL((bn_bwd_apply_kernel<false>), dim3(ew_grid(n8, true)), dim3(256), 0, s, (const uint16_t*)dout,
                       (const uint16_t*)outv, (const uint16_t*)ya, ca, (const uint16_t*)nullptr, (const float*)nullptr,
                       (uint16_t*)dya, (uint16_t*)nullptr, (uint16_t*)dz_out, n8, C8, C, msc, msh,
                       (const uint8_t*)omask);
  SDX_LAUNCH_CHECK();
  return hipSuccess;
}
```

Baseline: 22290 images/sec.

## Fuse BN stat reduction, finalize and apply into self-reducing kernels for fwd and bwd

Adds bn_apply_self and bn_bwd_apply_self kernels. Each block reduces the per-tile conv statistic slab for its 64 channels in LDS, computes BN scale/shift (or the backward coefficients) locally, then applies BN, ReLU, the residual and the mask over its own chunk of rows. In ResNet blocks this replaces the separate col_reduce/finalize launches and the later apply launch on the conv1/conv2/conv3/shortcut paths, whenever a plan marks the shape eligible and there is no cross-device comm. Every block in a channel group re-reduces the same slab, so reduction work is duplicated, and large slabs may need more LDS, which can lower occupancy.

```diff
diff --git a/csrc/bindings/block_ops.cpp b/csrc/bindings/block_ops.cpp
--- a/csrc/bindings/block_ops.cpp
+++ b/csrc/bindings/block_ops.cpp
@@ -178,7 +178,18 @@
   auto relu_bn = [](const torch::Tensor& y, const BnState& s) {
     return bn_apply(y, s.sc, s.sh, {}, true, c10::nullopt);
   };
-  std::vector<BnState> st;
+  std::vector<BnState> st(w.size());
+  auto fwd_in = [&](int i, const torch::Tensor& slab, double count) {
+    return BnFwdIn{slab, count, bn[i * 4], bn[i * 4 + 1], bn[i * 4 + 2], bn[i * 4 + 3]};
+  };
+  auto conv_bn_relu = [&](const torch::Tensor& in, int i, int64_t s, int64_t p) -> std::pair<torch::Tensor, torch::Tensor> {
+    auto c = conv_fwd(in, w[i], s, p, training, -1, c10::nullopt, c10::nullopt);
+    if (bn_self_ok(c[1], c[0], training, comm, false))
+      return {c[0], bn_forward_apply(c[0], fwd_in(i, c[1], rows_of(c[0])), nullptr, {}, 0, true, c10::nullopt, eps,
+                                     momentum, &st[i], nullptr)};
+    st[i] = bn_fwd(i, c[1], rows_of(c[0]));
+    return {c[0], relu_bn(c[0], st[i])};
+  };
   std::vector<torch::Tensor> out(kMask);
   torch::Tensor ys_side, slab_side;
   hipEvent_t sc_done = nullptr;
@@ -199,34 +210,46 @@
     sc_done = stream_mark();
   }
   const int64_t s1 = bottleneck ? 1 : stride, p1 = bottleneck ? 0 : 1;
-  auto c1 = conv_bn(x, 0, s1, p1);
-  st.push_back(c1.second);
-  auto a1 = relu_bn(c1.first, st[0]);
+  auto c1 = conv_bn_relu(x, 0, s1, p1);
+  const torch::Tensor& a1 = c1.second;
   const int64_t s2 = bottleneck ? stride : 1;
-  auto c2 = conv_bn(a1, 1, s2, 1);
-  st.push_back(c2.second);
-  torch::Tensor last = c2.first, a2;
+  torch::Tensor last, last_slab, a2, y2;
   int lastbn = 1;
+  auto conv_last = [&](const torch::Tensor& in, int i, int64_t s, int64_t p) {
+    auto c = conv_fwd(in, w[i], s, p, training, -1, c10::nullopt, c10::nullopt);
+    last = c[0];
+    if (bn_self_ok(c[1], c[0], training, comm, false))
+      last_slab = c[1];
+    else
+      st[i] = bn_fwd(i, c[1], rows_of(c[0]));
+  };
+  if (bottleneck) {
+    auto c2 = conv_bn_relu(a1, 1, s2, 1);
+    y2 = c2.first;
+    a2 = c2.second;
+  } else {
+    conv_last(a1, 1, s2, 1);
+    y2 = last;
+  }
   fold_fwd = fold_fwd && bottleneck && training && w[2].size(1) == 1 && w[2].size(2) == 1 &&
              (proj || (stride == 1 && w[2].size(0) == x.size(3))) && sdx_plan::fwd_bnapply_supported(knobs());
   torch::Tensor o, ys;
   auto shortcut = [&] {
     if (sc_done != nullptr) {
       stream_wait(sc_done);
-      st.push_back(bn_fwd(nconv, slab_side, rows_of(ys_side)));
+      st[nconv] = bn_fwd(nconv, slab_side, rows_of(ys_side));
       ys = ys_side;
     } else {
       auto cs = conv_bn(x, nconv, stride, 0);
-      st.push_back(cs.second);
+      st[nconv] = cs.second;
       ys = cs.first;
     }
   };
   torch::Tensor omask;
   if (bottleneck) {
-    a2 = relu_bn(c2.first, st[1]);
     if (fold_fwd) {
       auto c3s = conv_fwd(a2, w[2], 1, 0, true, -1, c10::nullopt, c10::nullopt, nullptr, true);
-      st.push_back(bn_fwd(2, c3s[1], rows_of(a2)));
+      st[2] = bn_fwd(2, c3s[1], rows_of(a2));
       GemmEpi epi{};
       epi.bn_scale = st[2].sc.data_ptr<float>();
       epi.bn_shift = st[2].sh.data_ptr<float>();
@@ -246,9 +269,7 @@
       o = conv_fwd(a2, w[2], 1, 0, false, -1, c10::nullopt, c10::nullopt, &epi)[0];
       last = torch::Tensor();
     } else {
-      auto c3 = conv_bn(a2, 2, 1, 0);
-      st.push_back(c3.second);
-      last = c3.first;
+      conv_last(a2, 2, 1, 0);
     }
     lastbn = 2;
   }
@@ -257,8 +278,33 @@
   const OptT om = training ? OptT(omask) : OptT();
   if (fold_fwd) {
   } else if (proj) {
-    shortcut();
-    o = bn_apply(last, st[lastbn].sc, st[lastbn].sh, {ys, st[nconv].sc, st[nconv].sh, 1}, true, om);
+    torch::Tensor ys_slab;
+    if (last_slab.defined()) {
+      if (sc_done != nullptr) {
+        stream_wait(sc_done);
+        ys = ys_side;
+        ys_slab = slab_side;
+      } else {
+        auto cs = conv_fwd(x, w[nconv], stride, 0, training, -1, c10::nullopt, c10::nullopt);
+        ys = cs[0];
+        ys_slab = cs[1];
+      }
+      if (bn_self_ok(ys_slab, ys, training, comm, false) && ys.sizes() == last.sizes()) {
+        const BnFwdIn b = fwd_in(nconv, ys_slab, rows_of(ys));
+        o = bn_forward_apply(last, fwd_in(lastbn, last_slab, rows_of(last)), &b, ys, 1, true, om, eps, momentum,
+                             &st[lastbn], &st[nconv]);
+      } else {
+        st[lastbn] = bn_fwd(lastbn, last_slab, rows_of(last));
+        st[nconv] = bn_fwd(nconv, ys_slab, rows_of(ys));
+      }
+    } else {
+      shortcut();
+    }
+    if (!o.defined())
+      o = bn_apply(last, st[lastbn].sc, st[lastbn].sh, {ys, st[nconv].sc, st[nconv].sh, 1}, true, om);
+  } else if (last_slab.defined()) {
+    o = bn_forward_apply(last, fwd_in(lastbn, last_slab, rows_of(last)), nullptr, x, 2, true, om, eps, momentum,
+                         &st[lastbn], nullptr);
   } else {
     o = bn_apply(last, st[lastbn].sc, st[lastbn].sh, {x, {}, {}, 2}, true, om);
   }
@@ -266,7 +312,7 @@
   out[kOut] = o;
   out[kY1] = c1.first;
   out[kA1] = a1;
-  out[kY2] = c2.first;
+  out[kY2] = y2;
   out[kA2] = bottleneck ? a2 : torch::Tensor();
   out[kY3] = bottleneck ? last : torch::Tensor();
   out[kYs] = ys;
@@ -330,9 +376,19 @@
   }
   {
     const BnBwdSrc src{dout, out, ylast, proj ? OptT(ys) : OptT()};
-    auto c = bn_bwd_coefs(comm, have_slab ? nullptr : &src, have_slab ? &*in_slab : nullptr, cnt_last, bset(lastbn),
-                          proj ? bset(nconv) : BnBwdSet{});
-    if (fold) {
+    const bool self = have_slab && !fold && bn_self_ok(*in_slab, dout, true, comm, true);
+    std::vector<torch::Tensor> c;
+    if (!self)
+      c = bn_bwd_coefs(comm, have_slab ? nullptr : &src, have_slab ? &*in_slab : nullptr, cnt_last, bset(lastbn),
+                       proj ? bset(nconv) : BnBwdSet{});
+    if (self) {
+      const bool bitmask = out.scalar_type() == at::kByte;
+      auto r = bn_bwd_coefs_apply(*in_slab, cnt_last, bset(lastbn), proj ? bset(nconv) : BnBwdSet{}, src,
+                                  !proj && !bitmask);
+      dylast = r[0];
+      if (proj) dys = r[1];
+      else if (!bitmask) dz = r[2];
+    } else if (fold) {
       coef3 = c[0];
       dz = dout;
       if (fold_sc)
@@ -365,26 +421,36 @@
   auto bn_relu_bwd = [&](const torch::Tensor& da, const torch::Tensor& y, const torch::Tensor& coef, int i) {
     return bn_bwd_apply({da, {}, y, {}, S(i, kSc), S(i, kSh)}, coef, c10::nullopt, false)[0];
   };
+  auto dgrad_bn_dy = [&](const torch::Tensor& dyo, const torch::Tensor& w, const torch::Tensor& y, int64_t st,
+                         int64_t pad, int i, double cnt, const DgradOpts& o = {}) -> torch::Tensor {
+    if (dgrad_bnstat_enabled()) {
+      DgradStat ds;
+      ds.ya = y; ds.ma = S(i, kMu); ds.msc = S(i, kSc); ds.msh = S(i, kSh);
+      auto r = conv_dgrad_bnstat(dyo, w, y.size(1), y.size(2), st, pad, -1, o, ds);
+      if (bn_self_ok(r[1], r[0], true, comm, true))
+        return bn_bwd_coefs_apply(r[1], cnt, bset(i), {}, {r[0], {}, y, {}, S(i, kSc), S(i, kSh)}, false)[0];
+      return bn_relu_bwd(r[0], y, bn_bwd_coefs(comm, nullptr, &r[1], cnt, bset(i))[0], i);
+    }
+    auto r = dgrad_bn(dyo, w, y, st, pad, i, cnt, o);
+    return bn_relu_bwd(r.first, y, r.second, i);
+  };
   torch::Tensor dy1;
   if (bottleneck) {
-    std::pair<torch::Tensor, torch::Tensor> r2;
+    torch::Tensor dy2;
     if (fold) {
       auto op = fold_dgrad_operands(coef3, fold_w[0], wt[2], a2, S(lastbn, kMu), gram3);
       side_fold_wgrad(dz, a2, fold_w[0], coef3, dw[2], side, gram3, Gfold.defined() ? &Gfold : nullptr);
-      r2 = dgrad_bn(dz, op.w, y2, 1, 0, 1, cnt_last, op.dgrad_opts(a2));
+      dy2 = dgrad_bn_dy(dz, op.w, y2, 1, 0, 1, cnt_last, op.dgrad_opts(a2));
     } else {
       side_wgrad(dylast, a2, 1, 1, 1, 0, dw[2], side);
-      r2 = dgrad_bn(dylast, wt[2], y2, 1, 0, 1, cnt_last);
-    }
-    auto dy2 = bn_relu_bwd(r2.first, y2, r2.second, 1);
+      dy2 = dgrad_bn_dy(dylast, wt[2], y2, 1, 0, 1, cnt_last);
+    }
     side_wgrad(dy2, a1, 3, 3, stride, 1, dw[1], side);
-    auto r1 = dgrad_bn(dy2, wt[1], y1, stride, 1, 0, cnt1);
-    dy1 = bn_relu_bwd(r1.first, y1, r1.second, 0);
+    dy1 = dgrad_bn_dy(dy2, wt[1], y1, stride, 1, 0, cnt1);
     side_wgrad(dy1, x, 1, 1, 1, 0, dw[0], side);
   } else {
     side_wgrad(dylast, a1, 3, 3, 1, 1, dw[1], side);
-    auto r1 = dgrad_bn(dylast, wt[1], y1, 1, 1, 0, cnt1);
-    dy1 = bn_relu_bwd(r1.first, y1, r1.second, 0);
+    dy1 = dgrad_bn_dy(dylast, wt[1], y1, 1, 1, 0, cnt1);
     side_wgrad(dy1, x, 3, 3, stride, 1, dw[0], side);
   }
   const int64_t s1 = bottleneck ? 1 : stride, p1 = bottleneck ? 0 : 1;
diff --git a/csrc/bindings/bn_ops.cpp b/csrc/bindings/bn_ops.cpp
--- a/csrc/bindings/bn_ops.cpp
+++ b/csrc/bindings/bn_ops.cpp
@@ -1,6 +1,7 @@
 #include "ops_decl.h"
 #include "conv_internal.h"
 #include "launchers.h"
+#include "bn_plan.h"
 
 #include <map>
 #include <mutex>
@@ -199,6 +200,63 @@
   check_hip(launch_bn_apply(y.data_ptr(), scale.data_ptr<float>(), shift.data_ptr<float>(), rp, s2, t2, (int)res.mode,
                             relu ? 1 : 0, out.data_ptr(), y.numel(), C, cur_stream(), mp),
             "bn_apply");
+  return out;
+}
+
+bool bn_self_ok(const torch::Tensor& slab, const torch::Tensor& y, bool training, int64_t comm, bool bwd) {
+  if (!training || comm != 0 || !slab.defined() || slab.dim() != 3 || y.dim() != 4) return false;
+  const int64_t C = y.size(3);
+  if (slab.size(2) != C || slab.size(0) >= (1 << 30) || slab.scalar_type() != at::kFloat || !slab.is_contiguous() ||
+      reinterpret_cast<uintptr_t>(slab.data_ptr()) % 16 != 0)
+    return false;
+  return bn_self_eligible((int)slab.size(0), (int)slab.size(1), (int)C, y.numel(), bwd);
+}
+
+torch::Tensor bn_forward_apply(const torch::Tensor& y, const BnFwdIn& a, const BnFwdIn* b, const OptT& r,
+                               int64_t res_mode, bool relu, OptT mask_out, double eps, double mom, BnState* st,
+                               BnState* st2, std::vector<torch::Tensor>* sums, int ew_blocks) {
+  check_bf16_nhwc(y, "y");
+  const int64_t C = y.size(3);
+  check_slab(a.slab, 2);
+  TORCH_CHECK(res_mode >= 0 && res_mode <= 2 && (res_mode == 1) == (b != nullptr), "bn_forward_apply: res_mode");
+  TORCH_CHECK(bn_self_ok(a.slab, y, true, 0, false), "bn_forward_apply: BN not eligible (bn_plan.h)");
+  const void* rp = nullptr;
+  if (res_mode != 0) {
+    TORCH_CHECK(r.has_value(), "residual tensor required");
+    check_bf16_nhwc(*r, "residual");
+    TORCH_CHECK(r->sizes() == y.sizes(), "residual shape mismatch");
+    rp = r->data_ptr();
+  }
+  c10::DeviceGuard dg(y.device());
+  FinalizeOut oa, ob;
+  const BnFinalizeArgs fa = finalize_args(y, C, a.count, a.g, a.b, eps, mom, true, a.rm, a.rv, oa);
+  auto sa = torch::empty({2, C}, y.options().dtype(at::kDouble));
+  BnFinalizeArgs fb{};
+  torch::Tensor sb;
+  if (b != nullptr) {
+    check_slab(b->slab, 2);
+    TORCH_CHECK(bn_self_ok(b->slab, y, true, 0, false), "bn_forward_apply: second BN not eligible (bn_plan.h)");
+    fb = finalize_args(y, C, b->count, b->g, b->b, eps, mom, true, b->rm, b->rv, ob);
+    sb = torch::empty({2, C}, y.options().dtype(at::kDouble));
+  }
+  auto out = torch::empty_like(y);
+  void* mp = nullptr;
+  if (mask_out.has_value()) {
+    check_mask(*mask_out, y.numel(), "mask_out");
+    mp = mask_out->data_ptr();
+  }
+  check_hip(launch_bn_apply_self(a.slab.data_ptr<float>(), (int)a.slab.size(0), sa.data_ptr<double>(), fa,
+                                 b ? b->slab.data_ptr<float>() : nullptr, b ? (int)b->slab.size(0) : 0,
+                                 b ? sb.data_ptr<double>() : nullptr, b ? &fb : nullptr, y.data_ptr(), rp,
+                                 (int)res_mode, relu ? 1 : 0, out.data_ptr(), y.numel(), (int)C, cur_stream(), mp,
+                                 ew_blocks),
+            "bn_apply_self");
+  if (st) *st = {oa.scale, oa.shift, oa.mean, oa.invstd};
+  if (st2 && b) *st2 = {ob.scale, ob.shift, ob.mean, ob.invstd};
+  if (sums) {
+    sums->push_back(sa);
+    if (b) sums->push_back(sb);
+  }
   return out;
 }
 
@@ -415,6 +473,41 @@
   return {dya, dyb, dz};
 }
 
+std::vector<torch::Tensor> bn_bwd_coefs_apply(const torch::Tensor& slab, double count, const BnBwdSet& sa,
+                                              const BnBwdSet& sb, const BnBwdSrc& s, bool want_dz, int ew_blocks) {
+  const torch::Tensor& dout = s.dout;
+  check_bf16_nhwc(dout, "dout");
+  check_bf16_nhwc(s.ya, "ya");
+  TORCH_CHECK(s.ya.sizes() == dout.sizes(), "ya shape");
+  BwdIn in;
+  in.C = dout.size(3);
+  mask_source(s, &in.op, &in.om);
+  if (s.yb.has_value()) {
+    check_bf16_nhwc(*s.yb, "yb");
+    TORCH_CHECK(s.yb->sizes() == dout.sizes(), "yb shape");
+    in.ybp = s.yb->data_ptr();
+  }
+  in_bn_ptrs(s.msc, s.msh, in.C, &in.mk_s, &in.mk_t);
+  const int64_t C = in.C;
+  const int nsum = in.nsum();
+  check_slab(slab, nsum);
+  TORCH_CHECK(slab.size(2) == C, "slab channels");
+  TORCH_CHECK(bn_self_ok(slab, dout, true, 0, true), "bn_bwd_coefs_apply: BN not eligible (bn_plan.h)");
+  c10::DeviceGuard dg(dout.device());
+  auto sums = torch::empty({nsum, C}, dout.options().dtype(at::kDouble));
+  CoefOut o;
+  const BnCoefArgs a = coef_args(dout, C, nsum - 1, count, sa, sb, o, 1.0);
+  auto dya = torch::empty_like(dout);
+  auto dyb = in.ybp ? torch::empty_like(dout) : torch::empty({0}, dout.options());
+  auto dz = want_dz ? torch::empty_like(dout) : torch::empty({0}, dout.options());
+  check_hip(launch_bn_bwd_apply_self(slab.data_ptr<float>(), (int)slab.size(0), nsum, sums.data_ptr<double>(), a,
+                                     dout.data_ptr(), in.op, s.ya.data_ptr(), in.ybp, dya.data_ptr(),
+                                     in.ybp ? dyb.data_ptr() : nullptr, want_dz ? dz.data_ptr() : nullptr,
+                                     dout.numel(), (int)C, cur_stream(), in.mk_s, in.mk_t, in.om, ew_blocks),
+            "bn_bwd_apply_self");
+  return {dya, dyb, dz, o.coef_a, o.coef_b, o.dga, o.dba, o.dgb, o.dbb, sums};
+}
+
 namespace {
 
 torch::Tensor syncbn_exchange_sums(int64_t comm, torch::Tensor slab) {
@@ -514,6 +607,68 @@
         pybind11::arg("mean_b") = pybind11::none(), pybind11::arg("inv_b") = pybind11::none(),
         pybind11::arg("sink_ga") = pybind11::none(), pybind11::arg("sink_ba") = pybind11::none(),
         pybind11::arg("sink_gb") = pybind11::none(), pybind11::arg("sink_bb") = pybind11::none());
+  m.def("bn_self_reduce_plan",
+        [](int64_t rows_slab, int64_t nsets, int64_t C, int64_t numel, int64_t comm, bool training, int64_t cap_kb,
+           int64_t ew_cap) {
+          const auto p = sdx_plan::bn_self_reduce_plan(rows_slab, (int)nsets, C, numel, comm, training,
+                                                       cap_kb < 0 ? sdx_plan::bn_self_cap_kb() : cap_kb, ew_cap);
+          return pybind11::make_tuple(p.self, p.groups, p.chunks, p.chunk_rows, p.slice_bytes);
+        },
+        "host-only: (self, groups, chunks, chunk_rows, slice_bytes) of one BN; cap_kb < 0: SDX_BN_SELF_KB",
+        pybind11::arg("rows_slab"), pybind11::arg("nsets"), pybind11::arg("C"), pybind11::arg("numel"),
+        pybind11::arg("comm") = 0, pybind11::arg("training") = true, pybind11::arg("cap_kb") = -1,
+        pybind11::arg("ew_cap") = sdx_plan::kEwBlocksDefault);
+  m.def("bn_self_cap_set",
+        [](int64_t kb) {
+          const int64_t old = sdx_plan::bn_self_cap_mut();
+          sdx_plan::bn_self_cap_mut() = kb < 0 ? 0 : kb;
+          return old;
+        },
+        "set the slab-slice cap in KiB (0: off) between calls; returns the previous value");
+  m.def("bn_stats_finalize_apply",
+        [](T y, T slab, double count, OptT gamma, OptT beta, OptT rm, OptT rv, OptT r, int64_t res_mode, OptT slab2,
+           double count2, OptT gamma2, OptT beta2, OptT rm2, OptT rv2, bool relu, OptT mask_out, double eps,
+           double momentum, int64_t ew_blocks) {
+          const BnFwdIn a{slab, count, gamma, beta, rm, rv};
+          BnFwdIn b;
+          if (res_mode == 1) {
+            TORCH_CHECK(slab2.has_value(), "slab2 required for res_mode 1");
+            b = BnFwdIn{*slab2, count2, gamma2, beta2, rm2, rv2};
+          }
+          BnState sa, sb;
+          std::vector<T> sums;
+          auto out = bn_forward_apply(y, a, res_mode == 1 ? &b : nullptr, r, res_mode, relu, mask_out, eps, momentum,
+                                      &sa, &sb, &sums, (int)ew_blocks);
+          std::vector<T> res{out, sums[0], sa.sc, sa.sh, sa.mu, sa.iv};
+          if (res_mode == 1) res.insert(res.end(), {sums[1], sb.sc, sb.sh, sb.mu, sb.iv});
+          return res;
+        },
+        "bn_stats_finalize + bn_apply in one launch: [out, sums, scale, shift, mean, invstd (, the same of BN 2)]",
+        pybind11::arg("y"), pybind11::arg("slab"), pybind11::arg("count"), pybind11::arg("gamma"),
+        pybind11::arg("beta"), pybind11::arg("running_mean"), pybind11::arg("running_var"),
+        pybind11::arg("r") = pybind11::none(), pybind11::arg("res_mode") = 0, pybind11::arg("slab2") = pybind11::none(),
+        pybind11::arg("count2") = 1.0, pybind11::arg("gamma2") = pybind11::none(),
+        pybind11::arg("beta2") = pybind11::none(), pybind11::arg("running_mean2") = pybind11::none(),
+        pybind11::arg("running_var2") = pybind11::none(), pybind11::arg("relu") = true,
+        pybind11::arg("mask_out") = pybind11::none(), pybind11::arg("eps") = 1e-5, pybind11::arg("momentum") = 0.1,
+        pybind11::arg("ew_blocks") = 0);
+  m.def("bn_bwd_coef_slab_apply",
+        [](T slab, double count, OptT g_a, T mean_a, T inv_a, OptT g_b, OptT mean_b, OptT inv_b, OptT sink_ga,
+           OptT sink_ba, OptT sink_gb, OptT sink_bb, T dout, OptT outv, T ya, OptT yb, bool want_dz, OptT msc, OptT msh,
+           int64_t ew_blocks) {
+          return bn_bwd_coefs_apply(slab, count, {g_a, mean_a, inv_a, sink_ga, sink_ba},
+                                    {g_b, mean_b, inv_b, sink_gb, sink_bb}, BnBwdSrc{dout, outv, ya, yb, msc, msh},
+                                    want_dz, (int)ew_blocks);
+        },
+        "bn_bwd_coef_slab + bn_bwd_apply in one launch: [dya, dyb, dz, coef_a, coef_b, dga, dba, dgb, dbb, sums]",
+        pybind11::arg("slab"), pybind11::arg("count"), pybind11::arg("g_a"), pybind11::arg("mean_a"),
+        pybind11::arg("inv_a"), pybind11::arg("g_b") = pybind11::none(), pybind11::arg("mean_b") = pybind11::none(),
+        pybind11::arg("inv_b") = pybind11::none(), pybind11::arg("sink_ga") = pybind11::none(),
+        pybind11::arg("sink_ba") = pybind11::none(), pybind11::arg("sink_gb") = pybind11::none(),
+        pybind11::arg("sink_bb") = pybind11::none(), pybind11::arg("dout"), pybind11::arg("outv") = pybind11::none(),
+        pybind11::arg("ya"), pybind11::arg("yb") = pybind11::none(), pybind11::arg("want_dz") = false,
+        pybind11::arg("msc") = pybind11::none(), pybind11::arg("msh") = pybind11::none(),
+        pybind11::arg("ew_blocks") = 0);
   m.def("bn_bwd_apply",
         [](T dout, OptT outv, T ya, T ca, OptT yb, OptT cb, bool want_dz, OptT msc, OptT msh) {
           return bn_bwd_apply(BnBwdSrc{dout, outv, ya, yb, msc, msh}, ca, cb, want_dz);
diff --git a/csrc/include/bn_epilogue.h b/csrc/include/bn_epilogue.h
--- a/csrc/include/bn_epilogue.h
+++ b/csrc/include/bn_epilogue.h
@@ -3,24 +3,26 @@
 
 namespace sdx {
 __device__ __forceinline__ void bn_finalize_one(int c, double s1, double s2, const BnFinalizeArgs& a) {
+#pragma clang fp contract(off)
   const double mean = s1 / a.count;
-  double var = s2 / a.count - mean * mean;
+  double var = __builtin_fma(-mean, mean, s2 / a.count);
   if (var < 0.0) var = 0.0;
   const float invstd = (float)(1.0 / sqrt(var + (double)a.eps));
   const float g = a.gamma ? a.gamma[c] : 1.f;
   const float b = a.beta ? a.beta[c] : 0.f;
   a.scale[c] = g * invstd;
-  a.shift[c] = b - (float)mean * g * invstd;
+  a.shift[c] = __builtin_fmaf(-((float)mean * g), invstd, b);
   a.mean[c] = (float)mean;
   a.invstd[c] = invstd;
   if (a.update_running) {
     const double unbiased = a.count > 1.0 ? var * a.count / (a.count - 1.0) : var;
     a.running_mean[c] = (1.f - a.momentum) * a.running_mean[c] + a.momentum * (float)mean;
-    a.running_var[c] = (1.f - a.momentum) * a.running_var[c] + a.momentum * (float)unbiased;
+    a.running_var[c] = __builtin_fmaf(a.momentum, (float)unbiased, (1.f - a.momentum) * a.running_var[c]);
   }
 }
 
 __device__ __forceinline__ void bn_coef_one(int c, int C, const double* s, int nsets, const BnCoefArgs& a) {
+#pragma clang fp contract(off)
   const double sdz = s[0];
   for (int set = 0; set < nsets; ++set) {
     const float* gg = set == 0 ? a.g_a : a.g_b;
@@ -32,7 +34,7 @@
     const double A = gam * inv;
     const double m1 = sdz / a.count, m2 = sdzy / a.count;
     const double D = -A * inv * inv * m2;
-    const double E = -A * m1 - D * mu;
+    const double E = __builtin_fma(-A, m1, -(D * mu));
     coef[c] = (float)A;
     coef[C + c] = (float)D;
     coef[2 * C + c] = (float)E;
diff --git a/csrc/include/bn_plan.h b/csrc/include/bn_plan.h
--- /dev/null
+++ b/csrc/include/bn_plan.h
@@ -0,0 +1,56 @@
+#pragma once
+#include <stdint.h>
+
+#include "conv_plan.h"
+
+namespace sdx_plan {
+
+constexpr int kBnSelfGroup = 64;
+constexpr int kBnSelfRowsPerPass = 32;
+constexpr int64_t kBnSelfKbDefault = 0;
+constexpr int64_t kBnSelfMaxKb = 64;
+constexpr int64_t kEwBlocksDefault = 2048;
+
+inline int64_t ew_blocks(int64_t n8, int64_t cap = kEwBlocksDefault, int64_t unroll = 1) {
+  int64_t g = cdiv(n8, 256 * unroll);
+  if (g > cap) g = cap;
+  return g < 1 ? 1 : g;
+}
+
+inline int64_t& bn_self_cap_mut() {
+  static int64_t kb = [] {
+    const long long v = env_int("SDX_BN_SELF_KB", kBnSelfKbDefault);
+    return (int64_t)(v < 0 ? 0 : v);
+  }();
+  return kb;
+}
+inline int64_t bn_self_cap_kb() { return bn_self_cap_mut(); }
+
+struct BnSelfPlan {
+  bool self = false;
+  int groups = 0;
+  int chunks = 0;
+  int64_t chunk_rows = 0;
+  int64_t slice_bytes = 0;
+};
+
+inline BnSelfPlan bn_self_reduce_plan(int64_t rows_slab, int nsets, int64_t C, int64_t numel, int64_t comm,
+                                      bool training, int64_t cap_kb, int64_t ew_cap = kEwBlocksDefault) {
+  BnSelfPlan p;
+  if (!training || comm != 0 || cap_kb <= 0) return p;
+  if (rows_slab < 1 || nsets < 2 || nsets > 3 || C < kBnSelfGroup || C % kBnSelfGroup != 0) return p;
+  if (numel < C || numel % C != 0 || numel / 8 >= (int64_t(1) << 31)) return p;
+  p.slice_bytes = rows_slab * nsets * kBnSelfGroup * 4;
+  if (p.slice_bytes > (cap_kb < kBnSelfMaxKb ? cap_kb : kBnSelfMaxKb) * 1024) return p;
+  const int64_t rows = numel / C;
+  p.groups = (int)(C / kBnSelfGroup);
+  int64_t chunks = ew_blocks(numel / 8, ew_cap) / p.groups;
+  if (chunks < 1) chunks = 1;
+  if (chunks > rows) chunks = rows;
+  p.chunk_rows = cdiv(rows, chunks);
+  p.chunks = (int)cdiv(rows, p.chunk_rows);
+  p.self = true;
+  return p;
+}
+
+}
diff --git a/csrc/include/conv_internal.h b/csrc/include/conv_internal.h
--- a/csrc/include/conv_internal.h
+++ b/csrc/include/conv_internal.h
@@ -71,6 +71,15 @@
 };
 torch::Tensor bn_apply(torch::Tensor y, torch::Tensor scale, torch::Tensor shift, const BnResidual& res, bool relu,
                        OptT mask_out);
+bool bn_self_ok(const torch::Tensor& slab, const torch::Tensor& y, bool training, int64_t comm, bool bwd);
+struct BnFwdIn {
+  torch::Tensor slab;
+  double count;
+  OptT g, b, rm, rv;
+};
+torch::Tensor bn_forward_apply(const torch::Tensor& y, const BnFwdIn& a, const BnFwdIn* b, const OptT& r,
+                               int64_t res_mode, bool relu, OptT mask_out, double eps, double mom, BnState* st,
+                               BnState* st2, std::vector<torch::Tensor>* sums = nullptr, int ew_blocks = 0);
 struct BnBwdSet {
   OptT gamma, mean, invstd, dgamma_sink, dbeta_sink;
 };
@@ -83,6 +92,8 @@
 std::vector<torch::Tensor> bn_bwd_coefs(int64_t comm, const BnBwdSrc* src, const torch::Tensor* slab, double count,
                                         const BnBwdSet& a, const BnBwdSet& b = {});
 std::vector<torch::Tensor> bn_bwd_apply(const BnBwdSrc& s, torch::Tensor ca, OptT cb, bool want_dz);
+std::vector<torch::Tensor> bn_bwd_coefs_apply(const torch::Tensor& slab, double count, const BnBwdSet& a,
+                                              const BnBwdSet& b, const BnBwdSrc& s, bool want_dz, int ew_blocks = 0);
 
 std::vector<torch::Tensor>& side_stash();
 hipEvent_t stream_mark();
diff --git a/csrc/include/launchers.h b/csrc/include/launchers.h
--- a/csrc/include/launchers.h
+++ b/csrc/include/launchers.h
@@ -185,6 +185,16 @@
 hipError_t launch_bn_bwd_apply(const void* dout, const void* outv, const void* ya, const float* ca, const void* yb,
                                const float* cb, void* dya, void* dyb, void* dz_out, long numel, int C, hipStream_t s,
                                const float* msc = nullptr, const float* msh = nullptr, const void* omask = nullptr);
+bool bn_self_eligible(int rows_slab, int nsets, int C, long numel, bool bwd);
+hipError_t launch_bn_apply_self(const float* slab, int rows_slab, double* sums, const BnFinalizeArgs& fa,
+                                const float* slab2, int rows_slab2, double* sums2, const BnFinalizeArgs* fb,
+                                const void* y, const void* r, int res_mode, int relu, void* out, long numel, int C,
+                                hipStream_t s, void* mask_out = nullptr, int ew_blocks = 0);
+hipError_t launch_bn_bwd_apply_self(const float* slab, int rows_slab, int nsets, double* sums, const BnCoefArgs& ca,
+                                    const void* dout, const void* outv, const void* ya, const void* yb, void* dya,
+                                    void* dyb, void* dz_out, long numel, int C, hipStream_t s,
+                                    const float* msc = nullptr, const float* msh = nullptr,
+                                    const void* omask = nullptr, int ew_blocks = 0);
 
 hipError_t launch_gpu_augment(const uint8_t* data, const int64_t* idx, int B, int H, int W, int S, int n_views,
                               uint64_t seed, const float* mean, const float* std, float scale_lo, float scale_hi,
diff --git a/csrc/kernels/bn.hip b/csrc/kernels/bn.hip
--- a/csrc/kernels/bn.hip
+++ b/csrc/kernels/bn.hip
@@ -3,6 +3,7 @@
 #include "common.h"
 #include "launchers.h"
 #include "bn_epilogue.h"
+#include "bn_plan.h"
 
 using namespace sdx;
 
@@ -84,6 +85,61 @@
   return true;
 }
 
+template <int NS>
+__device__ __forceinline__ void col_range_sum(const float* __restrict__ slab, int r0, int r1, int ty, int c, int C,
+                                              double (&acc)[NS]) {
+#pragma unroll
+  for (int q = 0; q < NS; ++q) acc[q] = 0.0;
+  if (c < C) {
+    constexpr int U = SDX_CR_UNROLL;
+    int r = r0 + ty;
+    for (; r + 4 * (U - 1) < r1; r += 4 * U) {
+      float v[U][NS];
+#pragma unroll
+      for (int u = 0; u < U; ++u)
+#pragma unroll
+        for (int q = 0; q < NS; ++q) v[u][q] = slab[((size_t)(r + 4 * u) * NS + q) * C + c];
+#pragma unroll
+      for (int u = 0; u < U; ++u)
+#pragma unroll
+        for (int q = 0; q < NS; ++q) acc[q] += (double)v[u][q];
+    }
+    for (; r < r1; r += 4)
+#pragma unroll
+      for (int q = 0; q < NS; ++q) acc[q] += (double)slab[((size_t)r * NS + q) * C + c];
+  }
+}
+__device__ __forceinline__ double col_fold4(const double (&red)[4][64], int tx) {
+  return red[0][tx] + red[1][tx] + red[2][tx] + red[3][tx];
+}
+
+template <int NS>
+__device__ __forceinline__ void col_reduce_block(const float* __restrict__ slab, int rows, int gy, int c, int C,
+                                                 double (&red)[2][NS][4][64], double (&t)[NS]) {
+  const int tx = threadIdx.x & 63, ty = threadIdx.x >> 6;
+  const int per = (rows + gy - 1) / gy;
+#pragma unroll
+  for (int q = 0; q < NS; ++q) t[q] = 0.0;
+  for (int y = 0; y < gy; ++y) {
+    const int r0 = y * per, r1 = min(rows, r0 + per);
+    double acc[NS];
+    col_range_sum<NS>(slab, r0, r1, ty, c, C, acc);
+#pragma unroll
+    for (int q = 0; q < NS; ++q) red[y & 1][q][ty][tx] = acc[q];
+    __syncthreads();
+    if (ty == (y & 3)) {
+#pragma unroll
+      for (int q = 0; q < NS; ++q) t[q] += col_fold4(red[y & 1][q], tx);
+    }
+  }
+  __syncthreads();
+#pragma unroll
+  for (int q = 0; q < NS; ++q) red[0][q][ty][tx] = t[q];
+  __syncthreads();
+#pragma unroll
+  for (int q = 0; q < NS; ++q) t[q] = col_fold4(red[0][q], tx);
+}
+
 template <int NS, int EPI, int XG>
 __global__ __launch_bounds__(256) void col_reduce_kernel(const float* __restrict__ slab, int rows, int C,
                                                          double* scratch, unsigned* counters,
@@ -103,26 +159,7 @@
   const int per = (rows + gy - 1) / gy;
   const int r0 = blockIdx.y * per, r1 = min(rows, r0 + per);
   double acc[NS];
-#pragma unroll
-  for (int q = 0; q < NS; ++q) acc[q] = 0.0;
-  if (c < C) {
-    constexpr int U = SDX_CR_UNROLL;
-    int r = r0 + ty;
-    for (; r + 4 * (U - 1) < r1; r += 4 * U) {
-      float v[U][NS];
-#pragma unroll
-      for (int u = 0; u < U; ++u)
-#pragma unroll
-        for (int q = 0; q < NS; ++q) v[u][q] = slab[((size_t)(r + 4 * u) * NS + q) * C + c];
-#pragma unroll
-      for (int u = 0; u < U; ++u)
-#pragma unroll
-        for (int q = 0; q < NS; ++q) acc[q] += (double)v[u][q];
-    }
-    for (; r < r1; r += 4)
-#pragma unroll
-      for (int q = 0; q < NS; ++q) acc[q] += (double)slab[((size_t)r * NS + q) * C + c];
-  }
+  col_range_sum<NS>(slab, r0, r1, ty, c, C, acc);
 #pragma unroll
   for (int q = 0; q < NS; ++q) red[q][ty][tx] = acc[q];
   __syncthreads();
@@ -130,7 +167,7 @@
   if (ty == 0 && c < C) {
 #pragma unroll
     for (int q = 0; q < NS; ++q) {
-      const double v = red[q][0][tx] + red[q][1][tx] + red[q][2][tx] + red[q][3][tx];
+      const double v = col_fold4(red[q], tx);
       __hip_atomic_store(sc + ((size_t)blockIdx.y * NS + q) * C + c, (unsigned long long)__double_as_longlong(v),
                          __ATOMIC_RELAXED, __HIP_MEMORY_SCOPE_AGENT);
     }
@@ -175,7 +212,7 @@
   }
   double t[NS];
 #pragma unroll
-  for (int q = 0; q < NS; ++q) t[q] = red[q][0][tx] + red[q][1][tx] + red[q][2][tx] + red[q][3][tx];
+  for (int q = 0; q < NS; ++q) t[q] = col_fold4(red[q], tx);
   bool go = true;
   if constexpr (XG != 0) go = xg_exchange<NS, XG>(t, c, C, xg, XG == 2 ? vz : xg.me);
   if (go && ty == 0 && c < C && vz == 0) {
@@ -513,6 +550,168 @@
   if (g > cap) g = cap;
   if (g < 1) g = 1;
   return (int)g;
+}
+
+struct BnSelfSlab {
+  const float* slab;
+  int rows, gy;
+  double* sums;
+};
+
+extern __shared__ __align__(16) float self_stage[];
+
+template <int NS>
+__device__ __forceinline__ void self_stage_in(const float* __restrict__ slab, int rows, int C, int c0, float* stage) {
+  constexpr int U = 8;
+  const int n4 = rows * NS * 16;
+  const float4* src = reinterpret_cast<const float4*>(slab + c0);
+  float4* dst = reinterpret_cast<float4*>(stage);
+  const int C4 = C >> 2;
+  for (int j0 = threadIdx.x; j0 < n4; j0 += 256 * U) {
+    float4 v[U];
+#pragma unroll
+    for (int u = 0; u < U; ++u) {
+      const int j = min(j0 + 256 * u, n4 - 1);
+      v[u] = src[(size_t)(j >> 4) * C4 + (j & 15)];
+    }
+#pragma unroll
+    for (int u = 0; u < U; ++u) {
+      const int j = j0 + 256 * u;
+      if (j < n4) dst[j] = v[u];
+    }
+  }
+  __syncthreads();
+}
+
+template <int RES, bool RELU>
+__global__ __launch_bounds__(256) void bn_apply_self_kernel(BnSelfSlab sa, BnFinalizeArgs fa, BnSelfSlab sb,
+                                                            BnFinalizeArgs fb, const uint16_t* __restrict__ y,
+                                                            const uint16_t* __restrict__ r,
+                                                            uint16_t* __restrict__ out, int rows, int chunk_rows,
+                                                            int C, uint8_t* __restrict__ mask_out) {
+  constexpr int NB = RES == 1 ? 2 : 1;
+  __shared__ double red[2][2][4][64];
+  __shared__ __align__(16) float aff[NB][4][64];
+  const int tx = threadIdx.x & 63, ty = threadIdx.x >> 6;
+  const int c0 = blockIdx.x * 64, c = c0 + tx;
+  const bool first = blockIdx.y == 0;
+#pragma unroll
+  for (int b = 0; b < NB; ++b) {
+    const BnSelfSlab& s = b == 0 ? sa : sb;
+    const BnFinalizeArgs& g = b == 0 ? fa : fb;
+    double t[2];
+    self_stage_in<2>(s.slab, s.rows, C, c0, self_stage);
+    col_reduce_block<2>(self_stage, s.rows, s.gy, tx, 64, red, t);
+    if (ty == 0) {
+      BnFinalizeArgs l = g;
+      l.gamma = g.gamma ? g.gamma + c0 : nullptr;
+      l.beta = g.beta ? g.beta + c0 : nullptr;
+      l.update_running = first ? g.update_running : 0;
+      l.running_mean = g.update_running ? g.running_mean + c0 : nullptr;
+      l.running_var = g.update_running ? g.running_var + c0 : nullptr;
+      l.scale = aff[b][0]; l.shift = aff[b][1]; l.mean = aff[b][2]; l.invstd = aff[b][3];
+      bn_finalize_one(tx, t[0], t[1], l);
+      if (first) {
+        s.sums[c] = t[0];
+        s.sums[C + c] = t[1];
+        g.scale[c] = aff[b][0][tx]; g.shift[c] = aff[b][1][tx];
+        g.mean[c] = aff[b][2][tx]; g.invstd[c] = aff[b][3][tx];
+      }
+    }
+    __syncthreads();
+  }
+  const int lane = threadIdx.x & 7, C8 = C >> 3;
+  ApplyOp<RES, RELU> op;
+  op.load(aff[0][0], aff[0][1], aff[NB - 1][0], aff[NB - 1][1], lane * 8);
+  const uint4* Y = reinterpret_cast<const uint4*>(y);
+  const uint4* R = reinterpret_cast<const uint4*>(r);
+  uint4* O = reinterpret_cast<uint4*>(out);
+  const int r0 = blockIdx.y * chunk_rows, r1 = min(rows, r0 + chunk_rows);
+  const int col = blockIdx.x * 8 + lane;
+  for (int row = r0 + (int)(threadIdx.x >> 3); row < r1; row += 32) {
+    const int e = row * C8 + col;
+    const uint4 o = op.run(ld16s<SDX_NT_EW_LOAD != 0>(Y + e),
+                           RES != 0 ? ld16s<SDX_NT_EW_LOAD != 0>(R + e) : make_uint4(0, 0, 0, 0));
+    st16<SDX_NT_EW != 0>(O + e, o);
+    if (mask_out) mask_out[e] = relu_bits(o);
+  }
+}
+
+template <bool TWO>
+__global__ __launch_bounds__(256) void bn_bwd_apply_self_kernel(
+    BnSelfSlab sl, BnCoefArgs ka, const uint16_t* __restrict__ dout, const uint16_t* __restrict__ outv,
+    const uint16_t* __restrict__ ya, const uint16_t* __restrict__ yb, uint16_t* __restrict__ dya,
+    uint16_t* __restrict__ dyb, uint16_t* __restrict__ dz_out, int rows, int chunk_rows, int C,
+    const float* __restrict__ msc, const float* __restrict__ msh, const uint8_t* __restrict__ omask) {
+  constexpr int NS = TWO ? 3 : 2;
+  __shared__ double red[2][NS][4][64];
+  __shared__ __align__(16) float coef[2][3][64];
+  const int tx = threadIdx.x & 63, ty = threadIdx.x >> 6;
+  const int c0 = blockIdx.x * 64, c = c0 + tx;
+  const bool first = blockIdx.y == 0;
+  {
+    double t[NS];
+    self_stage_in<NS>(sl.slab, sl.rows, C, c0, self_stage);
+    col_reduce_block<NS>(self_stage, sl.rows, sl.gy, tx, 64, red, t);
+    if (ty == 0) {
+      BnCoefArgs l = ka;
+      l.g_a = ka.g_a ? ka.g_a + c0 : nullptr;
+      l.mean_a = ka.mean_a + c0;
+      l.inv_a = ka.inv_a + c0;
+      l.coef_a = coef[0][0];
+      l.dgamma_a = first && ka.dgamma_a ? ka.dgamma_a + c0 : nullptr;
+      l.dbeta_a = first && ka.dbeta_a ? ka.dbeta_a + c0 : nullptr;
+      if (TWO) {
+        l.g_b = ka.g_b ? ka.g_b + c0 : nullptr;
+        l.mean_b = ka.mean_b + c0;
+        l.inv_b = ka.inv_b + c0;
+        l.coef_b = coef[1][0];
+        l.dgamma_b = first && ka.dgamma_b ? ka.dgamma_b + c0 : nullptr;
+        l.dbeta_b = first && ka.dbeta_b ? ka.dbeta_b + c0 : nullptr;
+      }
+      bn_coef_one(tx, 64, t, NS - 1, l);
+      if (first) {
+#pragma unroll
+        for (int q = 0; q < NS; ++q) sl.sums[(size_t)q * C + c] = t[q];
+#pragma unroll
+        for (int q = 0; q < 3; ++q) {
+          ka.coef_a[q * C + c] = coef[0][q][tx];
+          if (TWO) ka.coef_b[q * C + c] = coef[1][q][tx];
+        }
+      }
+    }
+    __syncthreads();
+  }
+  const int lane = threadIdx.x & 7, C8 = C >> 3;
+  const int col = blockIdx.x * 8 + lane;
+  BwdApplyOp<TWO> op;
+  op.load(coef[0][0], coef[1][0], msc ? msc + c0 : nullptr, msh ? msh + c0 : nullptr, 64, lane * 8);
+  const uint4* D = reinterpret_cast<const uint4*>(dout);
+  const uint4* OV = reinterpret_cast<const uint4*>(outv);
+  const uint4* YA = reinterpret_cast<const uint4*>(ya);
+  const uint4* YB = reinterpret_cast<const uint4*>(yb);
+  uint4* DA = reinterpret_cast<uint4*>(dya);
+  uint4* DB = reinterpret_cast<uint4*>(dyb);
+  uint4* DZ = reinterpret_cast<uint4*>(dz_out);
+  const bool has_out = outv != nullptr;
+  const uint4 z = make_uint4(0, 0, 0, 0);
+  const int r0 = blockIdx.y * chunk_rows, r1 = min(rows, r0 + chunk_rows);
+  for (int row = r0 + (int)(threadIdx.x >> 3); row < r1; row += 32) {
+    const int e = row * C8 + col;
+    float d[8];
+    uint4 ra, rb;
+    op.run(ld16s<SDX_NT_EW_LOAD != 0>(D + e), has_out ? ld16s<SDX_NT_EW_LOAD != 0>(OV + e) : z,
+           has_out, ld16s<SDX_NT_EW_LOAD != 0>(YA + e), TWO ? ld16s<SDX_NT_EW_LOAD != 0>(YB + e) : z, d, ra, rb,
+           omask, e);
+    if (DZ) st16<SDX_NT_EW != 0>(DZ + e, pack8(d));
+    st16<SDX_NT_EW != 0>(DA + e, ra);
+    if (TWO) st16<SDX_NT_EW != 0>(DB + e, rb);
+  }
+}
+
+sdx_plan::BnSelfPlan self_plan(int rows_slab, int nsets, int C, long numel, bool bwd, int ew_blocks = 0) {
+  return sdx_plan::bn_self_reduce_plan(rows_slab, nsets, C, numel, 0, true, sdx_plan::bn_self_cap_kb(),
+                                       ew_blocks > 0 ? ew_blocks : ew_grid(1L << 40, bwd));
 }
 
 }
@@ -658,3 +857,75 @@
   SDX_LAUNCH_CHECK();
   return hipSuccess;
 }
+
+namespace {
+hipError_t self_lds(const void* fn, size_t bytes) {
+  if (bytes + 16 * 1024 <= 64 * 1024) return hipSuccess;
+  return hipFuncSetAttribute(fn, hipFuncAttributeMaxDynamicSharedMemorySize, (int)(sdx_plan::kBnSelfMaxKb * 1024));
+}
+}
+
+bool bn_self_eligible(int rows_slab, int nsets, int C, long numel, bool bwd) {
+  return self_plan(rows_slab, nsets, C, numel, bwd).self;
+}
+
+hipError_t launch_bn_apply_self(const float* slab, int rows_slab, double* sums, const BnFinalizeArgs& fa,
+                                const float* slab2, int rows_slab2, double* sums2, const BnFinalizeArgs* fb,
+                                const void* y, const void* r, int res_mode, int relu, void* out, long numel, int C,
+                                hipStream_t s, void* mask_out, int ew_blocks) {
+  const sdx_plan::BnSelfPlan p = self_plan(rows_slab, 2, C, numel, false, ew_blocks);
+  if (!p.self || res_mode < 0 || res_mode > 2 || (res_mode != 0 && !r)) return hipErrorInvalidValue;
+  if (res_mode == 1 && (!slab2 || !sums2 || !fb || !self_plan(rows_slab2, 2, C, numel, false).self))
+    return hipErrorInvalidValue;
+  if (((uintptr_t)slab | (uintptr_t)slab2) % 16 != 0) return hipErrorInvalidValue;
+  const dim3 grid(p.groups, p.chunks), blk(256);
+  const size_t lds = (size_t)(res_mode == 1 && rows_slab2 > rows_slab ? rows_slab2 : rows_slab) * 2 * 64 * 4;
+  const BnSelfSlab sa{slab, rows_slab, col_reduce_gy(rows_slab), sums};
+  const BnSelfSlab sb = res_mode == 1 ? BnSelfSlab{slab2, rows_slab2, col_reduce_gy(rows_slab2), sums2} : BnSelfSlab{};
+  const BnFinalizeArgs f2 = res_mode == 1 ? *fb : BnFinalizeArgs{};
+  const uint16_t* yy = (const uint16_t*)y;
+  const uint16_t* rr = (const uint16_t*)r;
+  uint16_t* oo = (uint16_t*)out;
+  const int rows = (int)(numel / C), cr = (int)p.chunk_rows;
+#define SDX_APPLY_SELF(RM, RL)                                                                                     \
+  do {                                                                                                             \
+    if (hipError_t e = self_lds((const void*)bn_apply_self_kernel<RM, RL>, lds); e != hipSuccess) return e;        \
+    hipLaunchKernelGGL((bn_apply_self_kernel<RM, RL>), grid, blk, lds, s, sa, fa, sb, f2, yy, rr, oo, rows, cr, C, \
+                       (uint8_t*)mask_out);                                                                        \
+  } while (0)
+  if (res_mode == 0) { if (relu) SDX_APPLY_SELF(0, true); else SDX_APPLY_SELF(0, false); }
+  else if (res_mode == 1) { if (relu) SDX_APPLY_SELF(1, true); else SDX_APPLY_SELF(1, false); }
+  else { if (relu) SDX_APPLY_SELF(2, true); else SDX_APPLY_SELF(2, false); }
+#undef SDX_APPLY_SELF
+  SDX_LAUNCH_CHECK();
+  return hipSuccess;
+}
+
+hipError_t launch_bn_bwd_apply_self(const float* slab, int rows_slab, int nsets, double* sums, const BnCoefArgs& ca,
+                                    const void* dout, const void* outv, const void* ya, const void* yb, void* dya,
+                                    void* dyb, void* dz_out, long numel, int C, hipStream_t s, const float* msc,
+                                    const float* msh, const void* omask, int ew_blocks) {
+  const sdx_plan::BnSelfPlan p = self_plan(rows_slab, nsets, C, numel, true, ew_blocks);
+  if (!p.self || (nsets == 3) != (yb != nullptr) || (yb && (!dyb || !ca.coef_b || !ca.mean_b || !ca.inv_b)) ||
+      !ca.coef_a || !ca.mean_a || !ca.inv_a)
+    return hipErrorInvalidValue;
+  if ((uintptr_t)slab % 16 != 0) return hipErrorInvalidValue;
+  const dim3 grid(p.groups, p.chunks), blk(256);
+  const size_t lds = (size_t)p.slice_bytes;
+  const BnSelfSlab sl{slab, rows_slab, col_reduce_gy(rows_slab), sums};
+  const int rows = (int)(numel / C), cr = (int)p.chunk_rows;
+  if (hipError_t e = self_lds(yb ? (const void*)bn_bwd_apply_self_kernel<true>
+                                 : (const void*)bn_bwd_apply_self_kernel<false>, lds);
+      e != hipSuccess)
+    return e;
+  if (yb)
+    hipLaunchKernelGGL((bn_bwd_apply_self_kernel<true>), grid, blk, lds, s, sl, ca, (const uint16_t*)dout,
+                       (const uint16_t*)outv, (const uint16_t*)ya, (const uint16_t*)yb, (uint16_t*)dya, (uint16_t*)dyb,
+                       (uint16_t*)dz_out, rows, cr, C, msc, msh, (const uint8_t*)omask);
+  else
+    hipLaunchKernelGGL((bn_bwd_apply_self_kernel<false>), grid, blk, lds, s, sl, ca, (const uint16_t*)dout,
+                       (const uint16_t*)outv, (const uint16_t*)ya, (const uint16_t*)nullptr, (uint16_t*)dya,
+                       (uint16_t*)nullptr, (uint16_t*)dz_out, rows, cr, C, msc, msh, (const uint8_t*)omask);
+  SDX_LAUNCH_CHECK();
+  return hipSuccess;
+}
```

Measured after the change: 22260 images/sec. Within noise of the previous version (-0.1%).
